# xiexh20/VisTracker

Measured on AMD Instinct MI355X. Metric: frames/sec joint SMPL+object fit, higher is better.
Workload: dtype f32 (decoder GEMMs: 22-bit split-f16 operands x3 MFMA, fp32 accumulate)

## Files before the change

include/vistracker.h:

```cpp
#ifndef VISTRACKER_H
#define VISTRACKER_H

#ifdef __cplusplus
extern "C" {
#endif

#define VT_OK 0
#define VT_ERR_ARG -1
#define VT_ERR_HIP -2
#define VT_ERR_BUSY -3

#define VT_SMPL_V 6890
#define VT_SMPL_J 52
#define VT_SMPL_NB 10
#define VT_SMPL_NP 459
#define VT_FEAT 611
#define VT_HID 128

const char *vt_last_error(void);
int vt_version(void);

typedef struct vt_smplh vt_smplh;

int vt_smplh_create(vt_smplh **out, const float *v_template, const float *shapedirs, const float *posedirs,
                    const float *J_regressor, const float *weights, const int *parents, void *stream);
void vt_smplh_destroy(vt_smplh *h);

long vt_smplh_workspace_floats(int B);

int vt_smplh_forward(const vt_smplh *h, const float *pose, const float *betas, const float *trans, int B,
                     float *verts, float *jtr, float *v_posed, float *ws, void *stream);

long vt_smplh_bwd_scratch_floats(int B);
int vt_smplh_backward(const vt_smplh *h, const float *pose, const float *betas, int B, const float *dverts,
                      const float *djtr, const float *v_posed, const float *ws, float *scratch,
                      float *dpose, float *dbetas, float *dtrans, void *stream);

int vt_rodrigues_forward(const float *aa, int n, float *R, void *stream);
int vt_rodrigues_backward(const float *aa, int n, const float *dR, float *daa, void *stream);

typedef struct vt_landmarks vt_landmarks;
int vt_landmarks_create(vt_landmarks **out, const int *indptr, const int *indices, const float *data, int K, int V,
                        void *stream);
void vt_landmarks_destroy(vt_landmarks *h);
int vt_landmarks_forward(const vt_landmarks *h, const float *verts, int B, float *out, void *stream);
int vt_landmarks_backward(const vt_landmarks *h, const float *dout, int B, float *dverts, int accumulate, void *stream);

int vt_mahalanobis(const float *x, int B, int stride, int off, int n, const float *mean, const float *prec,
                   float *value, float *dx, float gscale, void *stream);

int vt_fill_f64(double *p, long n, double value, void *stream);
int vt_sum_to_term(const float *value, int n, float scale, double *term, void *stream);

typedef struct vt_sifnet vt_sifnet;
int vt_sifnet_create(vt_sifnet **out, const float *const *w, const float *const *b, const float *cam, void *stream);
void vt_sifnet_destroy(vt_sifnet *h);

int vt_nchw_to_nhwc(const float *src, int B, int C, int H, int W, float *dst, void *stream);

typedef struct {
    const float *maps[8];
    int res[8];
    const float *proj;
    int proj_cols;
    int act_level;
    int proj_level;
    int force_fp32;
} vt_maps;

int vt_query_forward(const vt_sifnet *h, const vt_maps *maps, const float *pts, const float *crop_center,
                     const float *body_center, int B, int N,
                     float *df, float *pca, float *parts, float *centers, float *vis, void *stream);
int vt_query_backward(const vt_sifnet *h, const vt_maps *maps, const float *pts, const float *crop_center,
                      const float *body_center, int B, int N,
                      const float *d_df, const float *d_pca, const float *d_parts, const float *d_centers,
                      const float *d_vis, float *dpts, void *stream);

long vt_query_projection_floats(const vt_maps *maps, int B);
int vt_query_build_projection(const vt_sifnet *h, const vt_maps *maps, int B, float *proj, void *stream);

int vt_query_human_loss(const vt_sifnet *h, const vt_maps *maps, const float *pts, const float *crop_center,
                        const float *body_center, int B, int N, const int *labels, const int *order, float w_dfh, float w_part,
                        float *dpts, double *terms, void *stream);
int vt_query_object_loss(const vt_sifnet *h, const vt_maps *maps, const float *pts, const float *crop_center,
                         const float *body_center, int B, int N, const float *occ, float w_obj,
                         float *dpts, double *terms, void *stream);

typedef struct vt_conv3x3 vt_conv3x3;
int vt_conv3x3_create(vt_conv3x3 **out, const float *weight, int cout, int cin, void *stream);
void vt_conv3x3_destroy(vt_conv3x3 *h);
int vt_conv3x3_forward(const vt_conv3x3 *h, const float *in, int B, int H, int W, float *out, int out_cstride, int out_coff, void *stream);
int vt_conv3x3_forward_gn(const vt_conv3x3 *h, const float *in, int in_cstride, int in_coff, const float *gn_stats, const float *gamma,
                          const float *beta, int groups, int B, int H, int W, float *out, int out_cstride, int out_coff, void *stream);
int vt_conv3x3_forward_gn_stats(const vt_conv3x3 *h, const float *in, int in_cstride, int in_coff, const float *gn_stats, const float *gamma,
                                const float *beta, int groups, int B, int H, int W, float *out, int out_cstride, int out_coff, double *stats_ws,
                                int stats_groups, void *stream);
int vt_conv3x3_forward_block(const vt_conv3x3 *h, const float *in, int in_cstride, int in_coff, const float *gn_stats, const float *gamma,
                             const float *beta, int groups, int B, int H, int W, float *out, int out_cstride, int out_coff,
                             const float *res, int res_cstride, int res_coff, float *fin, int fin_cstride, int fin_coff,
                             double *stats_ws, int stats_groups, void *stream);
int vt_conv3x3_tiles(int H, int W);
typedef struct vt_stem7x7 vt_stem7x7;
int vt_stem7x7_create(vt_stem7x7 **out, const float *weight, const float *bias, int cout, int cin, void *stream);
void vt_stem7x7_destroy(vt_stem7x7 *h);
int vt_stem7x7_forward(const vt_stem7x7 *h, const float *in, int in_cstride, int in_coff, int B, int H, int W, float *out, int out_cstride, int out_coff, void *stream);
typedef struct vt_conv1x1 vt_conv1x1;
int vt_conv1x1_create(vt_conv1x1 **out, const float *weight, const float *bias, int cout, int cin, void *stream);
void vt_conv1x1_destroy(vt_conv1x1 *h);
int vt_conv1x1_forward(const vt_conv1x1 *h, const float *in, int in_cstride, int in_coff, const float *gn_stats, const float *gamma, const float *beta, int groups,
                       int B, int H, int W, float *out, int out_cstride, int out_coff, const float *res, int res_cstride, int res_coff,
                       double *stats_ws, int stats_groups, void *stream);
int vt_groupnorm_finalize(double *ws, int nblk, int B, int HW, int C, int groups, float eps, void *stream);
int vt_conv3x3_forward_block_stats(const vt_conv3x3 *h, const float *in, int in_cstride, int in_coff, const float *gn_stats, const float *gamma,
                                   const float *beta, int groups, int B, int H, int W, float *out, int out_cstride, int out_coff,
                                   const float *res, int res_cstride, int res_coff, float *fin, int fin_cstride, int fin_coff,
                                   double *stats_ws, int stats_groups, double *fin_stats_ws, int fin_stats_groups, void *stream);
int vt_avgpool2x2_stats(const float *x, int B, int H, int W, int C, float *out, double *stats_ws, int stats_groups, void *stream);
int vt_sweep_blocks(int HW);
int vt_groupnorm_stats(const float *x, int cstride, int coff, int B, int HW, int C, int groups, float eps, double *ws, void *stream);

#define VT_PRECISION_SPLIT_F16 0
#define VT_PRECISION_FP32 1
int vt_sifnet_set_precision(vt_sifnet *h, int mode);
int vt_sifnet_get_precision(const vt_sifnet *h);

int vt_query_set_human_kernel(int threads);

int vt_query_project_step(const vt_sifnet *h, const vt_maps *maps, const float *pts, const float *crop_center,
                          const float *body_center, int B, int N, int df_idx, float threshold, float *pts_out,
                          float *df_target, void *stream);

int vt_kpts_step(const vt_landmarks *h, const float *verts, const float *kpts, const float *crop_center, int B, int mode, const float *cam, float net_size,
                 float gscale, double *term, float *J, float *dverts, int accumulate, void *stream);
int vt_query_human_step(const vt_sifnet *h, const vt_maps *maps, const float *pts, const float *crop_center, const float *body_center,
                        int B, int N, const int *labels, const int *order, float w_dfh, float w_part, int accumulate, float w_accel,
                        double *term_accel, float *dpts, double *terms, void *stream);
int vt_objstep_head(const float *M0, const float *noise, const float *t, const float *s, int B, const float *X0_points, int N, float *X_points,
                    const float *X0_verts, int NV, float *X_verts, float *R, double *terms, int nzero, float *svd_ws, void *stream);
int vt_temporal_loss2(const float *v, int B, int D, float gscale_accel, double *term_accel, float gscale_velocity, double *term_velocity, float *dv,
                      int init_zero, void *stream);
int vt_objstep_tail(const float *X0_verts, int NV, const float *dX_verts, const float *X0_points, int N, const float *dX_points, const float *s, int B,
                    const float *M0, const float *noise, const float *t, const float *t_init, float w_trans, double *term_trans,
                    float *dR, float *dt, float *dM,
                    float *pR, float *mR, float *vR, float lrR, float *pT, float *mT, float *vT, float lrT, int adam_step, float beta1, float beta2, float eps,
                    double *terms, const float *w, int nterms, float tol, int armed, float *state, int *stop_flag, float *history, int slot, int *ticket, int nzero,
                    float *svd_ws, void *stream);
int vt_objstep_tail_temporal(const float *X_points, float gscale_accel, double *term_accel, float gscale_velocity, double *term_velocity, int init_zero,
                             const float *X0_verts, int NV, const float *dX_verts, const float *X0_points, int N, const float *dX_points, const float *s, int B,
                             const float *M0, const float *noise, const float *t, const float *t_init, float w_trans, double *term_trans,
                             float *dR, float *dt, float *dM,
                             float *pR, float *mR, float *vR, float lrR, float *pT, float *mT, float *vT, float lrT, int adam_step, float beta1, float beta2, float eps,
                             double *terms, const float *w, int nterms, float tol, int armed, float *state, int *stop_flag, float *history, int slot, int *ticket, int nzero,
                             float *svd_ws, void *stream);
int vt_smplstep_tail(float *pose, const float *pose_init, float *dpose, int B, const float *prior_mean, const float *prior_prec, float gscale_prior,
                     double *term_prior, float w_pinit, double *term_pinit,
                     float *p0, int ps0, const float *g0, int gs0, float *m0, float *v0, int n0, float lr0,
                     float *p1, int ps1, const float *g1, int gs1, float *m1, float *v1, int n1, float lr1,
                     float *p2, int ps2, const float *g2, int gs2, float *m2, float *v2, int n2, float lr2,
                     int adam_step, float beta1, float beta2, float eps,
                     double *terms, const float *w, int nterms, float tol, int armed, float *state, int *stop_flag, float *history, int slot, int *ticket, int nzero,
                     void *stream);

int vt_so3_project_forward(const float *M0, const float *noise, int B, float *R, void *stream);
int vt_so3_project_backward(const float *M0, const float *noise, int B, const float *dR, float *dM, void *stream);

int vt_rigid_forward(const float *X0, int shared_x0, const float *R, const float *t, const float *s, int B, int N,
                     float *X, void *stream);
int vt_rigid_backward(const float *X0, int shared_x0, const float *s, int B, int N, const float *dX,
                      float *dR, float *dt, int accumulate, void *stream);

int vt_accel_loss(const float *v, int B, int D, const float *elem_w, float gscale, double *term, float *dv, void *stream);
int vt_accel_loss_strided(const float *v, int B, int D, int stride, const float *elem_w, float gscale, double *term,
                          float *dv, void *stream);
int vt_velocity_loss(const float *v, int B, int D, float gscale, double *term, float *dv, void *stream);

int vt_kpts_loss(const float *J, const float *kpts, const float *crop_center, int B, int K, int mode,
                 const float *cam, float net_size, float gscale, double *term, float *dJ, void *stream);

int vt_sqdiff_loss(const float *a, int a_stride, const float *b, int b_stride, int rows, int cols, float denom,
                   float gscale, double *term, float *da, void *stream);

long vt_collision_workspace_bytes(int B, int n_smpl_faces);
int vt_collision_loss(const float *smpl_verts, int n_smpl_verts, const int *smpl_faces, int n_smpl_faces, const float *obj_verts, int n_obj_verts,
                      const int *obj_faces, int n_obj_faces, int B, float sigma, int max_collisions, float gscale, double *term,
                      float *d_obj_t, int *pairs_per_frame, void *workspace, void *stream);

int vt_chamfer_ragged(const float *x, const int *offx, const float *y, const int *offy, int P, float gscale,
                      double *term, float *dx, float *dy, void *stream);
long vt_chamfer_ws_bytes(long total_x, long total_y, int P);
int vt_chamfer_ragged_ws(const float *x, const int *offx, long total_x, const float *y, const int *offy, long total_y, int P, float gscale,
                         double *term, float *dx, float *dy, void *ws, void *stream);

int vt_chamfer_ragged_idx(const float *x, const int *offx, long total_x, const float *y_base, const int *idx_y, const int *offy, long total_y, int P,
                          float gscale, double *term, float *dy_base, void *ws, int run_plan, void *stream);

int vt_nn_distance(const float *query, int nq, const float *search, int ns, int P, float *dist, void *stream);

long vt_sil_workspace_floats(int B, int NV, int NF, int size);
int vt_sil_forward(const float *verts, int B, int NV, const int *faces, int NF, const float *K, int size,
                   float *image, int *face_index, float *ws, void *stream);
int vt_sil_backward(const float *verts, int B, int NV, const int *faces, int NF, const float *K, int size,
                    const int *face_index, const float *d_image, float eps, float *ws, float *dverts, void *stream);
int vt_sil_setup(const float *mask_h, const float *mask_o, int B, int H, int W, const float *crop_centers, double expansion, int out, double crop_size,
                 double net_size, const double *cam_norm, double image_width, float *image_ref, float *keep_mask, float *K, double *boxes_ws, void *stream);

int vt_sil_mask_loss(const float *image, const float *keep, const float *ref, const float *occ, int B, int size,
                     float gscale, double *term, float *per_frame, float *d_image, void *stream);

int vt_sil_step(const float *verts, int B, int NV, const int *faces, int NF, const float *K, int size, const float *keep, const float *ref,
                const float *occ, float gscale, float eps, double *term, int *face_index, float *d_image, float *ws, float *dverts, void *stream);

int vt_triplane_render(const float *verts, const float *center, int B, int NV, const int *faces, int NF, int size,
                       float *masks, int *face_index, float *ws, void *stream);

int vt_upsample2x_bicubic_add(const float *low, const float *skip, int B, int h, int w, int C, float *out, void *stream);
int vt_upsample2x_bicubic_add_stats(const float *low, const float *skip, int B, int h, int w, int C, float *out, double *stats_ws, int stats_groups,
                                    void *stream);

long vt_groupnorm_workspace_doubles(int B, int HW, int C, int groups);
int vt_groupnorm_nhwc(const float *x, const float *gamma, const float *beta, int B, int HW, int C, int groups, float eps,
                      int relu, double *ws, float *y, void *stream);

int vt_adam_step(float *p, const float *g, float *m, float *v, long n, int step, float lr, float beta1, float beta2,
                 float eps, const int *stop_flag, void *stream);

int vt_adam_step_2d(float *p, long p_stride, const float *g, long g_stride, float *m, float *v, int rows, int cols,
                    int step, float lr, float beta1, float beta2, float eps, const int *stop_flag, void *stream);

int vt_loss_reduce_and_stop(const double *terms, const float *w, int nterms, float tol, int armed, float *state,
                            int *stop_flag, float *history, int slot, void *stream);

int vt_fill(float *p, long n, float value, void *stream);

int vt_stream_set_skip_flag(void *stream, const int *flag);

int vt_gen_round_compact(const float *surface, const float *df_target, const float *pre, const unsigned char *active, int B, int S, float filter_val,
                         float zmin, const long long *fill, int cap, int write, float *buf_points, int *order, float *kept_pre, long long *cnt,
                         long long *fill_out, void *stream);
int vt_gen_scatter_heads(const float *pred, int B, int C, int kmax, const long long *fill_old, const long long *cnt, int cap, float *buf, void *stream);
int vt_gen_resample(const float *samples, const int *order, const long long *cnt, const float *init, int B, int S, int S0, const float *u,
                    const float *pert, int M, float near_scale, float *out, void *stream);

long vt_render_workspace_bytes(int B, int NF, int size, int anti_aliasing, long list_entries);
int vt_render_static_create(void **layer, const float *verts, int NV, const int *faces, int NS, const float *face_colors, const float *K, float orig_size,
                            const float *light, int size, int anti_aliasing, void *stream);
void vt_render_static_destroy(void *layer);
int vt_render_rgb(const float *verts, int B, int NV, const int *faces, int NF, const float *face_colors, const float *K, int k_per_view, float orig_size,
                  const float *light, const float *background, const void *static_layer, int size, int anti_aliasing, float *rgb, float *alpha, float *depth,
                  int *face_index, void *ws, long ws_bytes, long *list_entries, void *stream);
int vt_render_panel_u8(const float *rgb, int B, int size, int row0, int nrows, int col0, int ncols, unsigned char *out, const long long *view_off,
                       long long out_row_stride, void *stream);
int vt_render_rgb_pv(const float *verts, int B, int NV, const int *faces, int NF, const float *face_colors, int colors_per_view, const float *K, int k_per_view,
                     float orig_size, const float *light, const float *background, const void *static_layer, int size, int anti_aliasing, float *rgb,
                     float *alpha, float *depth, int *face_index, void *ws, long ws_bytes, long *list_entries, void *stream);

int vt_contact_regions(const float *smpl_verts, const int *labels, const float *obj_verts, int B, int NVs, int NVo, int P, float thres, int *nn_idx,
                       float *nn_dist, int *part, int *count, float *centre, void *stream);
int vt_contact_spheres(const float *centre, const int *count, int B, int P, const float *unit_verts, int NSV, float radius, float *out, void *stream);
int vt_contact_face_colors(const int *part, int B, int NVo, const int *obj_faces, int NFo, int face_off, const float *base_colors, int NF, const float *palette,
                           int P, float *out, void *stream);

long vt_jpeg_workspace_bytes(int n, int H, int W, int subsampling, long long *max_out_bytes);
int vt_jpeg_encode(const unsigned char *rgb, int n, int H, int W, long long frame_stride, long long row_stride, int quality, int subsampling, void *ws,
                   long ws_bytes, unsigned char *out, long long out_cap, long long *offsets, void *stream);

int vt_query_set_clock_probe(unsigned long long *counters);
long vt_calibrate_workspace_bytes(void);
int vt_calibrate(void *work, double *out, void *stream);

#ifdef __cplusplus
}
#endif
#endif
```

vistracker_amd/_lib.py:

```python
from __future__ import annotations

import ctypes as C
import os

_HERE = os.path.dirname(os.path.abspath(__file__))
LIB_PATH = os.environ.get("VT_LIB_PATH", os.path.join(_HERE, "libvistracker_hip.so"))

vp = C.c_void_p
fp = C.c_void_p
ci = C.c_int
cl = C.c_long
cf = C.c_float
cd = C.c_double


class VtMaps(C.Structure):
    _fields_ = [("maps", C.c_void_p * 8), ("res", C.c_int * 8), ("proj", C.c_void_p), ("proj_cols", C.c_int),
                ("act_level", C.c_int), ("proj_level", C.c_int), ("force_fp32", C.c_int)]


SIGNATURES = {
    "vt_last_error": (C.c_char_p, []),
    "vt_version": (ci, []),
    "vt_smplh_create": (ci, [C.POINTER(vp), vp, vp, vp, vp, vp, vp, vp]),
    "vt_smplh_destroy": (None, [vp]),
    "vt_smplh_workspace_floats": (cl, [ci]),
    "vt_smplh_bwd_scratch_floats": (cl, [ci]),
    "vt_smplh_forward": (ci, [vp, fp, fp, fp, ci, fp, fp, fp, fp, vp]),
    "vt_smplh_backward": (ci, [vp, fp, fp, ci, fp, fp, fp, fp, fp, fp, fp, fp, vp]),
    "vt_rodrigues_forward": (ci, [fp, ci, fp, vp]),
    "vt_rodrigues_backward": (ci, [fp, ci, fp, fp, vp]),
    "vt_landmarks_create": (ci, [C.POINTER(vp), vp, vp, vp, ci, ci, vp]),
    "vt_landmarks_destroy": (None, [vp]),
    "vt_landmarks_forward": (ci, [vp, fp, ci, fp, vp]),
    "vt_landmarks_backward": (ci, [vp, fp, ci, fp, ci, vp]),
    "vt_mahalanobis": (ci, [fp, ci, ci, ci, ci, fp, fp, fp, fp, cf, vp]),
    "vt_fill_f64": (ci, [fp, cl, cd, vp]),
    "vt_sum_to_term": (ci, [fp, ci, cf, fp, vp]),
    "vt_sifnet_create": (ci, [C.POINTER(vp), C.POINTER(vp), C.POINTER(vp), vp, vp]),
    "vt_sifnet_destroy": (None, [vp]),
    "vt_nchw_to_nhwc": (ci, [fp, ci, ci, ci, ci, fp, vp]),
    "vt_query_forward": (ci, [vp, C.POINTER(VtMaps), fp, fp, fp, ci, ci, fp, fp, fp, fp, fp, vp]),
    "vt_query_backward": (ci, [vp, C.POINTER(VtMaps), fp, fp, fp, ci, ci, fp, fp, fp, fp, fp, fp, vp]),
    "vt_query_human_loss": (ci, [vp, C.POINTER(VtMaps), fp, fp, fp, ci, ci, fp, fp, cf, cf, fp, fp, vp]),
    "vt_query_object_loss": (ci, [vp, C.POINTER(VtMaps), fp, fp, fp, ci, ci, fp, cf, fp, fp, vp]),
    "vt_query_set_human_kernel": (ci, [ci]),
    "vt_sifnet_set_precision": (ci, [vp, ci]),
    "vt_sifnet_get_precision": (ci, [vp]),
    "vt_groupnorm_nhwc": (ci, [fp, fp, fp, ci, ci, ci, ci, cf, ci, fp, fp, vp]),
    "vt_upsample2x_bicubic_add": (ci, [fp, fp, ci, ci, ci, ci, fp, vp]),
    "vt_conv3x3_create": (ci, [C.POINTER(vp), vp, ci, ci, vp]),
    "vt_conv3x3_destroy": (None, [vp]),
    "vt_conv3x3_forward": (ci, [vp, fp, ci, ci, ci, fp, ci, ci, vp]),
    "vt_conv3x3_forward_gn": (ci, [vp, fp, ci, ci, fp, fp, fp, ci, ci, ci, ci, fp, ci, ci, vp]),
    "vt_groupnorm_stats": (ci, [fp, ci, ci, ci, ci, ci, ci, cf, fp, vp]),
    "vt_groupnorm_workspace_doubles": (C.c_long, [ci, ci, ci, ci]),
    "vt_groupnorm_finalize": (ci, [fp, ci, ci, ci, ci, ci, cf, vp]),
    "vt_conv3x3_tiles": (ci, [ci, ci]),
    "vt_kpts_step": (ci, [vp, fp, fp, fp, ci, ci, vp, cf, cf, fp, fp, fp, ci, vp]),
    "vt_query_human_step": (ci, [vp, C.POINTER(VtMaps), fp, fp, fp, ci, ci, fp, fp, cf, cf, ci, cf, fp, fp, fp, vp]),
    "vt_objstep_head": (ci, [fp, fp, fp, fp, ci, fp, ci, fp, fp, ci, fp, fp, fp, ci, fp, vp]),
    "vt_temporal_loss2": (ci, [fp, ci, ci, cf, fp, cf, fp, fp, ci, vp]),
    "vt_objstep_tail": (ci, [fp, ci, fp, fp, ci, fp, fp, ci, fp, fp, fp, fp, cf, fp, fp, fp, fp,
                             fp, fp, fp, cf, fp, fp, fp, cf, ci, cf, cf, cf,
                             fp, vp, ci, cf, ci, fp, fp, fp, ci, fp, ci, fp, vp]),
    "vt_objstep_tail_temporal": (ci, [fp, cf, fp, cf, fp, ci,
                                      fp, ci, fp, fp, ci, fp, fp, ci, fp, fp, fp, fp, cf, fp, fp, fp, fp,
                                      fp, fp, fp, cf, fp, fp, fp, cf, ci, cf, cf, cf,
                                      fp, vp, ci, cf, ci, fp, fp, fp, ci, fp, ci, fp, vp]),
    "vt_smplstep_tail": (ci, [fp, fp, fp, ci, fp, fp, cf, fp, cf, fp,
                              fp, ci, fp, ci, fp, fp, ci, cf, fp, ci, fp, ci, fp, fp, ci, cf, fp, ci, fp, ci, fp, fp, ci, cf, ci, cf, cf, cf,
                              fp, vp, ci, cf, ci, fp, fp, fp, ci, fp, ci, vp]),
    "vt_stream_set_skip_flag": (ci, [vp, vp]),
    "vt_conv1x1_create": (ci, [C.POINTER(vp), vp, vp, ci, ci, vp]),
    "vt_stem7x7_create": (ci, [C.POINTER(vp), vp, vp, ci, ci, vp]),
    "vt_stem7x7_destroy": (None, [vp]),
    "vt_stem7x7_forward": (ci, [vp, fp, ci, ci, ci, ci, ci, fp, ci, ci, vp]),
    "vt_conv1x1_destroy": (None, [vp]),
    "vt_conv1x1_forward": (ci, [vp, fp, ci, ci, fp, fp, fp, ci, ci, ci, ci, fp, ci, ci, fp, ci, ci, fp, ci, vp]),
    "vt_conv3x3_forward_block": (ci, [vp, fp, ci, ci, fp, fp, fp, ci, ci, ci, ci, fp, ci, ci, fp, ci, ci, fp, ci, ci, fp, ci, vp]),
    "vt_conv3x3_forward_block_stats": (ci, [vp, fp, ci, ci, fp, fp, fp, ci, ci, ci, ci, fp, ci, ci, fp, ci, ci, fp, ci, ci, fp, ci, fp, ci, vp]),
    "vt_avgpool2x2_stats": (ci, [fp, ci, ci, ci, ci, fp, fp, ci, vp]),
    "vt_sweep_blocks": (ci, [ci]),
    "vt_upsample2x_bicubic_add_stats": (ci, [fp, fp, ci, ci, ci, ci, fp, fp, ci, vp]),
    "vt_conv3x3_forward_gn_stats": (ci, [vp, fp, ci, ci, fp, fp, fp, ci, ci, ci, ci, fp, ci, ci, fp, ci, vp]),
    "vt_triplane_render": (ci, [fp, fp, ci, ci, fp, ci, ci, fp, fp, fp, vp]),
    "vt_query_project_step": (ci, [vp, C.POINTER(VtMaps), fp, fp, fp, ci, ci, ci, cf, fp, fp, vp]),
    "vt_query_projection_floats": (C.c_long, [C.POINTER(VtMaps), ci]),
    "vt_query_build_projection": (ci, [vp, C.POINTER(VtMaps), ci, fp, vp]),
    "vt_so3_project_forward": (ci, [fp, fp, ci, fp, vp]),
    "vt_so3_project_backward": (ci, [fp, fp, ci, fp, fp, vp]),
    "vt_rigid_forward": (ci, [fp, ci, fp, fp, fp, ci, ci, fp, vp]),
    "vt_rigid_backward": (ci, [fp, ci, fp, ci, ci, fp, fp, fp, ci, vp]),
    "vt_accel_loss": (ci, [fp, ci, ci, fp, cf, fp, fp, vp]),
    "vt_accel_loss_strided": (ci, [fp, ci, ci, ci, fp, cf, fp, fp, vp]),
    "vt_velocity_loss": (ci, [fp, ci, ci, cf, fp, fp, vp]),
    "vt_kpts_loss": (ci, [fp, fp, fp, ci, ci, ci, vp, cf, cf, fp, fp, vp]),
    "vt_sqdiff_loss": (ci, [fp, ci, fp, ci, ci, ci, cf, cf, fp, fp, vp]),
    "vt_chamfer_ragged": (ci, [fp, fp, fp, fp, ci, cf, fp, fp, fp, vp]),
    "vt_chamfer_ws_bytes": (C.c_long, [C.c_long, C.c_long, ci]),
    "vt_chamfer_ragged_ws": (ci, [fp, fp, C.c_long, fp, fp, C.c_long, ci, cf, fp, fp, fp, fp, vp]),
    "vt_chamfer_ragged_idx": (ci, [fp, fp, C.c_long, fp, fp, fp, C.c_long, ci, cf, fp, fp, fp, ci, vp]),
    "vt_collision_workspace_bytes": (cl, [ci, ci]),
    "vt_collision_loss": (ci, [fp, ci, fp, ci, fp, ci, fp, ci, ci, cf, ci, cf, fp, fp, fp, fp, vp]),
    "vt_nn_distance": (ci, [fp, ci, fp, ci, ci, fp, vp]),
    "vt_sil_workspace_floats": (cl, [ci, ci, ci, ci]),
    "vt_sil_forward": (ci, [fp, ci, ci, fp, ci, fp, ci, fp, fp, fp, vp]),
    "vt_sil_backward": (ci, [fp, ci, ci, fp, ci, fp, ci, fp, fp, cf, fp, fp, vp]),
    "vt_sil_mask_loss": (ci, [fp, fp, fp, fp, ci, ci, cf, fp, fp, fp, vp]),
    "vt_sil_step": (ci, [fp, ci, ci, fp, ci, fp, ci, fp, fp, fp, cf, cf, fp, fp, fp, fp, fp, vp]),
    "vt_gen_round_compact": (ci, [fp, fp, fp, vp, ci, ci, cf, cf, vp, ci, ci, fp, vp, fp, vp, vp, vp]),
    "vt_gen_scatter_heads": (ci, [fp, ci, ci, ci, vp, vp, ci, fp, vp]),
    "vt_gen_resample": (ci, [fp, vp, vp, fp, ci, ci, ci, fp, fp, ci, cf, fp, vp]),
    "vt_sil_setup": (ci, [fp, fp, ci, ci, ci, fp, C.c_double, ci, C.c_double, C.c_double, C.POINTER(C.c_double), C.c_double, fp, fp, fp, fp, vp]),
    "vt_adam_step": (ci, [fp, fp, fp, fp, cl, ci, cf, cf, cf, cf, fp, vp]),
    "vt_adam_step_2d": (ci, [fp, cl, fp, cl, fp, fp, ci, ci, ci, cf, cf, cf, cf, fp, vp]),
    "vt_loss_reduce_and_stop": (ci, [fp, vp, ci, cf, ci, fp, fp, fp, ci, vp]),
    "vt_fill": (ci, [fp, cl, cf, vp]),
    "vt_selftest_mfma": (ci, [fp, fp, fp, vp]),
    "vt_query_set_clock_probe": (ci, [vp]),
    "vt_render_workspace_bytes": (cl, [ci, ci, ci, ci, cl]),
    "vt_render_static_create": (ci, [C.POINTER(vp), fp, ci, fp, ci, fp, fp, cf, C.POINTER(cf), ci, ci, vp]),
    "vt_render_static_destroy": (None, [vp]),
    "vt_render_rgb": (ci, [fp, ci, ci, fp, ci, fp, fp, ci, cf, C.POINTER(cf), C.POINTER(cf), vp, ci, ci, fp, fp, fp, fp, fp, cl,
                           C.POINTER(cl), vp]),
    "vt_render_panel_u8": (ci, [fp, ci, ci, ci, ci, ci, ci, fp, fp, C.c_longlong, vp]),
    "vt_render_rgb_pv": (ci, [fp, ci, ci, fp, ci, fp, ci, fp, ci, cf, C.POINTER(cf), C.POINTER(cf), vp, ci, ci, fp, fp, fp, fp, fp, cl,
                              C.POINTER(cl), vp]),
    "vt_contact_regions": (ci, [fp, fp, fp, ci, ci, ci, ci, cf, fp, fp, fp, fp, fp, vp]),
    "vt_contact_spheres": (ci, [fp, fp, ci, ci, fp, ci, cf, fp, vp]),
    "vt_contact_face_colors": (ci, [fp, ci, ci, fp, ci, ci, fp, ci, fp, ci, fp, vp]),
    "vt_jpeg_workspace_bytes": (cl, [ci, ci, ci, ci, C.POINTER(C.c_longlong)]),
    "vt_jpeg_encode": (ci, [fp, ci, ci, ci, C.c_longlong, C.c_longlong, ci, ci, vp, cl, vp, C.c_longlong,
                            C.POINTER(C.c_longlong), vp]),
    "vt_calibrate_workspace_bytes": (cl, []),
    "vt_calibrate": (ci, [vp, C.POINTER(C.c_double), vp]),
}

_lib = None


class VtError(RuntimeError):
    pass


def lib():
    global _lib
    if _lib is None:
        if not os.path.exists(LIB_PATH):
            raise VtError(f"{LIB_PATH} is missing: build it with `make -C vistracker_amd/csrc` "
                          f"(or `python -c 'import __graft_entry__ as g; g.build()'`); there is no CPU fallback")
        import torch
        l = C.CDLL(LIB_PATH)
        for name, (res, args) in SIGNATURES.items():
            fn = getattr(l, name)
            fn.restype = res
            fn.argtypes = args
        _lib = l
        _host_tuning()
    return _lib


def _host_tuning():
    if os.environ.get("VT_HOST_THP", "keep") != "off":
        return
    try:
        C.CDLL(None, use_errno=True).prctl(41, 1, 0, 0, 0)
    except Exception:
        pass


VT_OK, VT_ERR_ARG, VT_ERR_HIP, VT_ERR_BUSY = 0, -1, -2, -3


def check(rc: int):
    if rc != 0:
        raise VtError(f"libvistracker_hip error {rc}: {lib().vt_last_error().decode()}")


def stream_ptr():
    import torch
    return torch.cuda.current_stream().cuda_stream


def dptr(t):
    if t is None:
        return None
    if not t.is_cuda:
        raise VtError("libvistracker_hip ops need CUDA (HIP) tensors; there is no CPU fallback in the product path")
    if not t.is_contiguous():
        raise VtError("libvistracker_hip ops need contiguous tensors")
    import torch
    if t.device.index != torch.cuda.current_device():
        raise VtError(f"tensor on cuda:{t.device.index} but the current device is cuda:{torch.cuda.current_device()}: "
                      "wrap the call in `with torch.cuda.device(tensor.device):`")
    return t.data_ptr()
```

vistracker_amd/csrc/smplh.hip:

```cpp
#include "common.h"
#include <cstring>

#define V_ VT_SMPL_V
#define J_ VT_SMPL_J
#define NB_ VT_SMPL_NB
#define NP_ VT_SMPL_NP
#define VP_ 6912
#define NVT_ 27
#define KQ_ 472
#define NQ_ 480
typedef float f32x4 __attribute__((ext_vector_type(4)));
#define MFMA16(a, b, c) __builtin_amdgcn_mfma_f32_16x16x4f32((a), (b), (c), 0, 0, 0)

#define WS_R 0
#define WS_J (52 * 9)
#define WS_G (WS_J + 52 * 3)
#define WS_A (WS_G + 52 * 12)
#define WS_FRAME (WS_A + 52 * 12)
#define PT_DA 0
#define PT_DTR 624
#define PT_N 627
#define KTOT_ (VP_ * 3)
#define KG_SLAB 24
#define NKS_ (KTOT_ / 16 / KG_SLAB)

#define SCHED_STEPS 32
#define SCHED_WIDTH 10
struct SmplParents { int p[J_]; int nsteps; short sched[SCHED_STEPS][SCHED_WIDTH]; };

#define SP_K 8
struct vt_smplh {
    float *Q_kcv, *Q_t, *W_jv, *W_v64, *J_t, *J_s;
    float *W_sp;
    int nnz;
    SmplParents par;
};

struct RodCtx { float n, ax, ay, az, c, s, qn, w, x, y, z; };

__device__ __forceinline__ void rodrigues_fwd(const float *t, float *R, RodCtx *k)
{
    const float xe = t[0] + 1e-8f, ye = t[1] + 1e-8f, ze = t[2] + 1e-8f;
    const float n = sqrtf(xe * xe + ye * ye + ze * ze);
    const float ax = t[0] / n, ay = t[1] / n, az = t[2] / n;
    const float h = n * 0.5f;
    const float c = cosf(h), s = sinf(h);
    const float q0 = c, q1 = s * ax, q2 = s * ay, q3 = s * az;
    const float qn = sqrtf(q0 * q0 + q1 * q1 + q2 * q2 + q3 * q3);
    const float w = q0 / qn, x = q1 / qn, y = q2 / qn, z = q3 / qn;
    const float w2 = w * w, x2 = x * x, y2 = y * y, z2 = z * z;
    const float wx = w * x, wy = w * y, wz = w * z, xy = x * y, xz = x * z, yz = y * z;
    R[0] = w2 + x2 - y2 - z2; R[1] = 2 * xy - 2 * wz;   R[2] = 2 * wy + 2 * xz;
    R[3] = 2 * wz + 2 * xy;   R[4] = w2 - x2 + y2 - z2; R[5] = 2 * yz - 2 * wx;
    R[6] = 2 * xz - 2 * wy;   R[7] = 2 * wx + 2 * yz;   R[8] = w2 - x2 - y2 + z2;
    if (k) { k->n = n; k->ax = ax; k->ay = ay; k->az = az; k->c = c; k->s = s; k->qn = qn; k->w = w; k->x = x; k->y = y; k->z = z; }
}

__device__ __forceinline__ void rodrigues_bwd(const float *t, const float *dR, float *dt)
{
    float R[9]; RodCtx k; rodrigues_fwd(t, R, &k);
    const float w = k.w, x = k.x, y = k.y, z = k.z;
    const float dw = 2 * w * (dR[0] + dR[4] + dR[8]) + 2 * (-z * dR[1] + y * dR[2] + z * dR[3] - x * dR[5] - y * dR[6] + x * dR[7]);
    const float dx = 2 * x * (dR[0] - dR[4] - dR[8]) + 2 * (y * dR[1] + z * dR[2] + y * dR[3] - w * dR[5] + z * dR[6] + w * dR[7]);
    const float dy = 2 * y * (-dR[0] + dR[4] - dR[8]) + 2 * (x * dR[1] + w * dR[2] + x * dR[3] + z * dR[5] - w * dR[6] + z * dR[7]);
    const float dz = 2 * z * (-dR[0] - dR[4] + dR[8]) + 2 * (-w * dR[1] + x * dR[2] + w * dR[3] + y * dR[5] + x * dR[6] + y * dR[7]);
    const float dot = w * dw + x * dx + y * dy + z * dz;
    const float dq0 = (dw - w * dot) / k.qn, dq1 = (dx - x * dot) / k.qn, dq2 = (dy - y * dot) / k.qn, dq3 = (dz - z * dot) / k.qn;
    const float dh = -k.s * dq0 + k.c * (k.ax * dq1 + k.ay * dq2 + k.az * dq3);
    const float dax = k.s * dq1, day = k.s * dq2, daz = k.s * dq3;
    const float dn = 0.5f * dh - (t[0] * dax + t[1] * day + t[2] * daz) / (k.n * k.n);
    dt[0] = dax / k.n + dn * (t[0] + 1e-8f) / k.n;
    dt[1] = day / k.n + dn * (t[1] + 1e-8f) / k.n;
    dt[2] = daz / k.n + dn * (t[2] + 1e-8f) / k.n;
}

__global__ void rodrigues_fwd_kernel(const float *aa, int n, float *R)
{
    const int i = blockIdx.x * blockDim.x + threadIdx.x;
    if (i >= n) return;
    float t[3] = {aa[3 * i], aa[3 * i + 1], aa[3 * i + 2]}, r[9];
    rodrigues_fwd(t, r, nullptr);
#pragma unroll
    for (int e = 0; e < 9; e++) R[9 * i + e] = r[e];
}

__global__ void rodrigues_bwd_kernel(const float *aa, int n, const float *dR, float *daa)
{
    const int i = blockIdx.x * blockDim.x + threadIdx.x;
    if (i >= n) return;
    float t[3] = {aa[3 * i], aa[3 * i + 1], aa[3 * i + 2]}, g[9], d[3];
#pragma unroll
    for (int e = 0; e < 9; e++) g[e] = dR[9 * i + e];
    rodrigues_bwd(t, g, d);
    daa[3 * i] = d[0]; daa[3 * i + 1] = d[1]; daa[3 * i + 2] = d[2];
}

__global__ __launch_bounds__(64) void smplh_pose_kernel(const float *__restrict__ pose, const float *__restrict__ betas,
                                                        const float *__restrict__ trans, const float *__restrict__ J_t,
                                                        const float *__restrict__ J_s, SmplParents par,
                                                        float *__restrict__ ws, float *__restrict__ jtr, const int *skip)
{
    VT_SKIP_RETURN(skip);
    __shared__ float sR[J_ * 9], sJ[J_ * 3], sG[J_ * 12];
    const int b = blockIdx.x, j = threadIdx.x;
    float *w = ws + (size_t)b * WS_FRAME;
    if (j < J_) {
        float t[3] = {pose[(b * J_ + j) * 3], pose[(b * J_ + j) * 3 + 1], pose[(b * J_ + j) * 3 + 2]}, R[9];
        rodrigues_fwd(t, R, nullptr);
#pragma unroll
        for (int e = 0; e < 9; e++) { sR[j * 9 + e] = R[e]; w[WS_R + j * 9 + e] = R[e]; }
#pragma unroll
        for (int c = 0; c < 3; c++) {
            float a = J_t[j * 3 + c];
#pragma unroll
            for (int l = 0; l < NB_; l++) a += J_s[(j * 3 + c) * NB_ + l] * betas[b * NB_ + l];
            sJ[j * 3 + c] = a; w[WS_J + j * 3 + c] = a;
        }
    }
    __shared__ int sPar[J_];
    if (j < J_) sPar[j] = par.p[j];
    __syncthreads();
    int lvl = 0, maxl = 0;
    if (j < J_) { for (int q = j; q != 0; q = sPar[q]) lvl++; }
    maxl = lvl;
    for (int o = 32; o > 0; o >>= 1) maxl = max(maxl, __shfl_xor(maxl, o, 64));
    maxl = __builtin_amdgcn_readfirstlane(maxl);
    if (j == 0) { for (int r = 0; r < 3; r++) { for (int c = 0; c < 3; c++) sG[r * 4 + c] = sR[r * 3 + c]; sG[r * 4 + 3] = sJ[r]; } }
    __syncthreads();
    for (int l = 1; l <= maxl; l++) {
        if (j < J_ && lvl == l) {
            const int i = j, p = sPar[i];
            const float *Gp = sG + 12 * p, *Ri = sR + 9 * i;
            const float d0 = sJ[3 * i] - sJ[3 * p], d1 = sJ[3 * i + 1] - sJ[3 * p + 1], d2 = sJ[3 * i + 2] - sJ[3 * p + 2];
            float *Gi = sG + 12 * i;
            for (int r = 0; r < 3; r++) {
                const float g0 = Gp[r * 4], g1 = Gp[r * 4 + 1], g2 = Gp[r * 4 + 2];
                Gi[r * 4 + 0] = g0 * Ri[0] + g1 * Ri[3] + g2 * Ri[6];
                Gi[r * 4 + 1] = g0 * Ri[1] + g1 * Ri[4] + g2 * Ri[7];
                Gi[r * 4 + 2] = g0 * Ri[2] + g1 * Ri[5] + g2 * Ri[8];
                Gi[r * 4 + 3] = g0 * d0 + g1 * d1 + g2 * d2 + Gp[r * 4 + 3];
            }
        }
        __syncthreads();
    }
    if (j < J_) {
        const float *G = sG + 12 * j;
#pragma unroll
        for (int r = 0; r < 3; r++) {
            const float gt = G[r * 4 + 3];
            w[WS_G + j * 12 + r * 4 + 0] = G[r * 4]; w[WS_G + j * 12 + r * 4 + 1] = G[r * 4 + 1];
            w[WS_G + j * 12 + r * 4 + 2] = G[r * 4 + 2]; w[WS_G + j * 12 + r * 4 + 3] = gt;
            w[WS_A + j * 12 + r * 4 + 0] = G[r * 4]; w[WS_A + j * 12 + r * 4 + 1] = G[r * 4 + 1]; w[WS_A + j * 12 + r * 4 + 2] = G[r * 4 + 2];
            w[WS_A + j * 12 + r * 4 + 3] = gt - (G[r * 4] * sJ[3 * j] + G[r * 4 + 1] * sJ[3 * j + 1] + G[r * 4 + 2] * sJ[3 * j + 2]);
            if (jtr) jtr[(b * J_ + j) * 3 + r] = gt + trans[3 * b + r];
        }
    }
}

#define FWD_FB 16
#ifndef FWD_PF
#define FWD_PF 6
#endif
#define AXS 516
#define SAS 628
#define FWD_R0 (FWD_FB * AXS > 8 * SAS ? FWD_FB * AXS : 8 * SAS)
__global__ __launch_bounds__(256) void smplh_verts_kernel(const float *__restrict__ Q_kcv, const float *__restrict__ W_jv,
                                                          const float *__restrict__ betas, const float *__restrict__ trans,
                                                          const float *__restrict__ ws, int B,
                                                          float *__restrict__ verts, float *__restrict__ v_posed, const float *__restrict__ W_sp, int nnz, const int *skip)
{
    VT_SKIP_RETURN(skip);
    extern __shared__ __attribute__((aligned(16))) float lds[];
    float *sAx = lds;
    float *sA = lds;
    float *sVp = lds + FWD_R0;
    float *sW = sVp + FWD_FB * 64 * 3;
    float *sTr = sW + (nnz > 0 ? 2 * SP_K * 64 : J_ * 64);
    const int tid = threadIdx.x, wave = tid >> 6, lane = tid & 63, q = lane >> 4, j = lane & 15;
    const int b0 = blockIdx.y * FWD_FB, v = blockIdx.x * 64 + wave * 16 + j;
    for (int k = tid; k < KQ_; k += 256) {
        const int e9 = k % 9;
        const float sub = (k < NP_ && (e9 == 0 || e9 == 4 || e9 == 8)) ? 1.f : 0.f;
        float val[FWD_FB];
#pragma unroll
        for (int f = 0; f < FWD_FB; f++) {
            const int b = min(b0 + f, B - 1);
            if (k < NP_) val[f] = ws[(size_t)b * WS_FRAME + WS_R + 9 + k];
            else if (k < NP_ + NB_) val[f] = betas[b * NB_ + (k - NP_)];
            else val[f] = (k == NP_ + NB_) ? 1.f : 0.f;
        }
#pragma unroll
        for (int f = 0; f < FWD_FB; f++) sAx[f * AXS + k] = val[f] - sub;
    }
    if (nnz > 0) {
        for (int i = tid; i < nnz * 64; i += 256) {
            sW[i] = W_sp[(size_t)(i >> 6) * VP_ + blockIdx.x * 64 + (i & 63)];
            sW[SP_K * 64 + i] = W_sp[(size_t)(SP_K + (i >> 6)) * VP_ + blockIdx.x * 64 + (i & 63)];
        }
    } else
        for (int i = tid; i < J_ * 64; i += 256) sW[i] = W_jv[(i >> 6) * VP_ + blockIdx.x * 64 + (i & 63)];
    if (tid < FWD_FB * 3) { const int f = tid / 3, b = min(b0 + f, B - 1); sTr[tid] = trans[b * 3 + tid % 3]; }
    __syncthreads();

    f32x4 acc[3];
#pragma unroll
    for (int c = 0; c < 3; c++) acc[c] = (f32x4){0.f, 0.f, 0.f, 0.f};
    constexpr int NS = KQ_ / 8;
    float bq[FWD_PF][2][3];
#define FWD_LOADQ(slot_, s_)                                                                     \
    {                                                                                            \
        const float *qk = Q_kcv + (size_t)(8 * (s_) + 2 * q) * 3 * VP_ + v;                      \
        _Pragma("unroll") for (int e = 0; e < 2; e++)                                            \
            _Pragma("unroll") for (int c = 0; c < 3; c++) bq[slot_][e][c] = qk[(size_t)(e * 3 + c) * VP_]; \
    }
#pragma unroll
    for (int s = 0; s < FWD_PF; s++) FWD_LOADQ(s, s)
#pragma unroll
    for (int s = 0; s < NS; s++) {
        const float2 av = *reinterpret_cast<const float2 *>(sAx + j * AXS + 8 * s + 2 * q);
#pragma unroll
        for (int c = 0; c < 3; c++) acc[c] = MFMA16(av.x, bq[s % FWD_PF][0][c], acc[c]);
#pragma unroll
        for (int c = 0; c < 3; c++) acc[c] = MFMA16(av.y, bq[s % FWD_PF][1][c], acc[c]);
        if (s + FWD_PF < NS) FWD_LOADQ(s % FWD_PF, s + FWD_PF)
        __builtin_amdgcn_sched_barrier(0);
    }
#undef FWD_LOADQ
    __syncthreads();
#pragma unroll
    for (int r = 0; r < 4; r++)
#pragma unroll
        for (int c = 0; c < 3; c++) sVp[((4 * q + r) * 64 + wave * 16 + j) * 3 + c] = acc[c][r];
    const int vv = tid & 63, vg = blockIdx.x * 64 + vv;
#pragma unroll 1
    for (int r = 0; r < 4; r++) {
        if ((r & 1) == 0) {
            if (r) __syncthreads();
            for (int i = tid; i < 8 * 624; i += 256) {
                const int sl = i / 624, f = 4 * (sl >> 1) + r + (sl & 1), b = min(b0 + f, B - 1);
                sA[sl * SAS + (i % 624)] = ws[(size_t)b * WS_FRAME + WS_A + (i % 624)];
            }
            __syncthreads();
        }
        const int f = 4 * wave + r, b = b0 + f;
        float T[12];
#pragma unroll
        for (int e = 0; e < 12; e++) T[e] = 0.f;
        const float4 *Af = reinterpret_cast<const float4 *>(sA + (2 * wave + (r & 1)) * SAS);
        if (nnz > 0) {
            for (int k = 0; k < nnz; k++) {
                const int jj = __float_as_int(sW[k * 64 + vv]);
                const float wj = sW[(SP_K + k) * 64 + vv];
                const float4 a0 = Af[jj * 3], a1 = Af[jj * 3 + 1], a2 = Af[jj * 3 + 2];
                T[0] += wj * a0.x; T[1] += wj * a0.y; T[2] += wj * a0.z; T[3] += wj * a0.w;
                T[4] += wj * a1.x; T[5] += wj * a1.y; T[6] += wj * a1.z; T[7] += wj * a1.w;
                T[8] += wj * a2.x; T[9] += wj * a2.y; T[10] += wj * a2.z; T[11] += wj * a2.w;
            }
        } else {
#pragma unroll 4
            for (int jj = 0; jj < J_; jj++) {
                const float wj = sW[jj * 64 + vv];
                const float4 a0 = Af[jj * 3], a1 = Af[jj * 3 + 1], a2 = Af[jj * 3 + 2];
                T[0] += wj * a0.x; T[1] += wj * a0.y; T[2] += wj * a0.z; T[3] += wj * a0.w;
                T[4] += wj * a1.x; T[5] += wj * a1.y; T[6] += wj * a1.z; T[7] += wj * a1.w;
                T[8] += wj * a2.x; T[9] += wj * a2.y; T[10] += wj * a2.z; T[11] += wj * a2.w;
            }
        }
        if (b < B && vg < V_) {
            const float p0 = sVp[(f * 64 + vv) * 3], p1 = sVp[(f * 64 + vv) * 3 + 1], p2 = sVp[(f * 64 + vv) * 3 + 2];
            const size_t o = ((size_t)b * V_ + vg) * 3;
#pragma unroll
            for (int rr = 0; rr < 3; rr++) verts[o + rr] = T[rr * 4] * p0 + T[rr * 4 + 1] * p1 + T[rr * 4 + 2] * p2 + T[rr * 4 + 3] + sTr[f * 3 + rr];
            v_posed[o] = p0; v_posed[o + 1] = p1; v_posed[o + 2] = p2;
        }
    }
}

template <int FB>
__global__ __launch_bounds__(256) void smplh_bwd_tile_kernel(const float *__restrict__ W_v64, const float *__restrict__ ws,
                                                             const float *__restrict__ v_posed, const float *__restrict__ dverts,
                                                             int B, float *__restrict__ part, float *__restrict__ dvp_g, const int *skip)
{
    VT_SKIP_RETURN(skip);
    extern __shared__ __attribute__((aligned(16))) float lds[];
    float *sdT = lds;
    float *sA = sdT + 256 * 13;
    const int tid = threadIdx.x, tile = blockIdx.x, b0 = blockIdx.y * FB, v0 = tile * 256, v = v0 + tid;
    const int wave = tid >> 6, lane = tid & 63, q = lane >> 4, j = lane & 15;
    for (int i = tid; i < FB * 624; i += 256) { const int f = i / 624, b = min(b0 + f, B - 1); sA[i] = ws[(size_t)b * WS_FRAME + WS_A + (i % 624)]; }
    float w1[4][13], w2[64];
#pragma unroll
    for (int mt = 0; mt < 4; mt++)
#pragma unroll
        for (int ks = 0; ks < 13; ks++) w1[mt][ks] = W_v64[(size_t)(v0 + 64 * wave + 16 * mt + j) * 64 + 4 * ks + q];
#pragma unroll
    for (int ks = 0; ks < 64; ks++) w2[ks] = W_v64[(size_t)(v0 + 4 * ks + q) * 64 + wave * 16 + j];
    __syncthreads();
    float dvn[3] = {0.f, 0.f, 0.f}, vpn[3] = {0.f, 0.f, 0.f};
    auto fetch = [&](int b) {
#pragma unroll
        for (int r = 0; r < 3; r++) { dvn[r] = 0.f; vpn[r] = 0.f; }
        if (b < B && v < V_) {
            const size_t o = ((size_t)b * V_ + v) * 3;
            dvn[0] = dverts[o]; dvn[1] = dverts[o + 1]; dvn[2] = dverts[o + 2];
            vpn[0] = v_posed[o]; vpn[1] = v_posed[o + 1]; vpn[2] = v_posed[o + 2];
        }
    };
    fetch(b0);
#pragma unroll 1
    for (int f = 0; f < FB; f++) {
        const int b = b0 + f;
        const float dv[3] = {dvn[0], dvn[1], dvn[2]}, vp[3] = {vpn[0], vpn[1], vpn[2]};
        if (f + 1 < FB) fetch(b + 1);
#pragma unroll
        for (int r = 0; r < 3; r++) {
            sdT[tid * 13 + r * 4 + 0] = dv[r] * vp[0]; sdT[tid * 13 + r * 4 + 1] = dv[r] * vp[1];
            sdT[tid * 13 + r * 4 + 2] = dv[r] * vp[2]; sdT[tid * 13 + r * 4 + 3] = dv[r];
        }
        __syncthreads();
        {
            f32x4 t[4];
#pragma unroll
            for (int mt = 0; mt < 4; mt++) t[mt] = (f32x4){0.f, 0.f, 0.f, 0.f};
#pragma unroll
            for (int ks = 0; ks < 13; ks++) {
                const float bv = j < 12 ? sA[f * 624 + (4 * ks + q) * 12 + j] : 0.f;
#pragma unroll
                for (int mt = 0; mt < 4; mt++) t[mt] = MFMA16(w1[mt][ks], bv, t[mt]);
            }
            const int r4 = (j < 12 ? (j >> 2) : 0) * 4 + 3;
#pragma unroll
            for (int mt = 0; mt < 4; mt++) {
#pragma unroll
                for (int r = 0; r < 4; r++) {
                    const int vl = 64 * wave + 16 * mt + 4 * q + r;
                    float x = t[mt][r] * sdT[vl * 13 + r4];
                    x += __shfl_down(x, 4, 16) + __shfl_down(x, 8, 16);
                    if (j < 3 && b < B) dvp_g[(size_t)b * KTOT_ + (size_t)(v0 + vl) * 3 + j] = x;
                }
            }
        }
        {
            f32x4 acc = (f32x4){0.f, 0.f, 0.f, 0.f}, acc2 = (f32x4){0.f, 0.f, 0.f, 0.f};
#pragma unroll
            for (int ks = 0; ks < 64; ks += 2) {
                const int va = 4 * ks + q, vb = va + 4;
                const float a0 = j < 12 ? sdT[va * 13 + j] : 0.f, a1 = j < 12 ? sdT[vb * 13 + j] : 0.f;
                acc = MFMA16(a0, w2[ks], acc);
                acc2 = MFMA16(a1, w2[ks + 1], acc2);
            }
            acc += acc2;
            if (b < B) {
                float *dst = part + ((size_t)tile * B + b) * PT_N;
                const int jn = wave * 16 + j;
#pragma unroll
                for (int r = 0; r < 4; r++) {
                    const int e = 4 * q + r;
                    if (e < 12) {
                        if (jn < J_) dst[PT_DA + jn * 12 + e] = acc[r];
                        else if (jn == J_ && (e & 3) == 3) dst[PT_DTR + (e >> 2)] = acc[r];
                    }
                }
            }
        }
        __syncthreads();
    }
}

#define BL_M 96
#ifndef BL_NW
#define BL_NW 1
#endif
#define BL_AS 132
__global__ __launch_bounds__(256) void smplh_bwd_blend_kernel(const float *__restrict__ Q_p, const float *__restrict__ dvp_g, int B,
                                                              float *__restrict__ part3, const int *skip)
{
    VT_SKIP_RETURN(skip);
    __shared__ __attribute__((aligned(16))) float sA[BL_M * BL_AS];
    const int tid = threadIdx.x, wave = tid >> 6, lane = tid & 63, q = lane >> 4, j = lane & 15;
    const int ks = blockIdx.x, m0 = blockIdx.z * BL_M, nt0 = blockIdx.y * (4 * BL_NW) + wave * BL_NW;
    f32x4 acc[6][BL_NW];
#pragma unroll
    for (int mt = 0; mt < 6; mt++)
#pragma unroll
        for (int n = 0; n < BL_NW; n++) acc[mt][n] = (f32x4){0.f, 0.f, 0.f, 0.f};
    const float4 *Q4 = reinterpret_cast<const float4 *>(Q_p);
#pragma unroll 1
    for (int c = 0; c < KG_SLAB / 8; c++) {
        __syncthreads();
        for (int i = tid; i < BL_M * 32; i += 256) {
            const int row = i >> 5, c4 = i & 31, b = m0 + row;
            float4 v = make_float4(0.f, 0.f, 0.f, 0.f);
            if (b < B) v = *reinterpret_cast<const float4 *>(dvp_g + (size_t)b * KTOT_ + (size_t)(ks * KG_SLAB + c * 8) * 16 + c4 * 4);
            *reinterpret_cast<float4 *>(sA + row * BL_AS + c4 * 4) = v;
        }
        __syncthreads();
#pragma unroll
        for (int g = 0; g < 8; g++) {
            const size_t kg = (size_t)ks * KG_SLAB + c * 8 + g;
            float bq[BL_NW][4];
#pragma unroll
            for (int n = 0; n < BL_NW; n++) {
                const float4 fq = Q4[(kg * (NQ_ / 16) + min(nt0 + n, NQ_ / 16 - 1)) * 64 + lane];
                bq[n][0] = fq.x; bq[n][1] = fq.y; bq[n][2] = fq.z; bq[n][3] = fq.w;
            }
#pragma unroll
            for (int mt = 0; mt < 6; mt++) {
                const float4 a4 = *reinterpret_cast<const float4 *>(sA + (mt * 16 + j) * BL_AS + g * 16 + q * 4);
                const float av[4] = {a4.x, a4.y, a4.z, a4.w};
#pragma unroll
                for (int s = 0; s < 4; s++)
#pragma unroll
                    for (int n = 0; n < BL_NW; n++) acc[mt][n] = MFMA16(av[s], bq[n][s], acc[mt][n]);
            }
        }
    }
#pragma unroll
    for (int mt = 0; mt < 6; mt++) {
#pragma unroll
        for (int r = 0; r < 4; r++) {
            const int b = m0 + mt * 16 + 4 * q + r;
            if (b < B) {
                float *dst = part3 + ((size_t)ks * B + b) * NQ_;
#pragma unroll
                for (int n = 0; n < BL_NW; n++)
                    if (nt0 + n < NQ_ / 16) dst[(nt0 + n) * 16 + j] = acc[mt][n][r];
            }
        }
    }
}

__global__ __launch_bounds__(256) void smplh_bwd_frame_kernel(const float *__restrict__ pose, const float *__restrict__ J_s,
                                                              SmplParents par, const float *__restrict__ ws,
                                                              const float *__restrict__ part, const float *__restrict__ part3,
                                                              const float *__restrict__ djtr, int B, float *__restrict__ dpose, float *__restrict__ dbetas,
                                                              float *__restrict__ dtrans, const int *skip)
{
    VT_SKIP_RETURN(skip);
    __shared__ float red[PT_N], red3[NQ_];
    __shared__ float sdG[J_ * 12], sdJ[J_ * 3], sdR[J_ * 9];
    __shared__ float sG[J_ * 12], sRm[J_ * 9], sJr[J_ * 3];
    const int b = blockIdx.x, tid = threadIdx.x;
    const float *w = ws + (size_t)b * WS_FRAME;
    for (int i = tid; i < J_ * 12; i += 256) sG[i] = w[WS_G + i];
    for (int i = tid; i < J_ * 9; i += 256) sRm[i] = w[WS_R + i];
    for (int i = tid; i < J_ * 3; i += 256) sJr[i] = w[WS_J + i];
    for (int i = tid; i < PT_N; i += 256) {
        float s = 0.f;
#pragma unroll 9
        for (int t = 0; t < NVT_; t++) s += part[((size_t)t * B + b) * PT_N + i];
        red[i] = s;
    }
    for (int i = tid; i < NQ_; i += 256) {
        float s = 0.f;
#pragma unroll 9
        for (int t = 0; t < NKS_; t++) s += part3[((size_t)t * B + b) * NQ_ + i];
        red3[i] = s;
    }
    __syncthreads();
    if (tid < J_) {
        const int j = tid;
        const float *G = sG + 12 * j; const float *Jr = sJr;
        float dj[3] = {0.f, 0.f, 0.f};
#pragma unroll
        for (int r = 0; r < 3; r++) {
            const float dat = red[PT_DA + 12 * j + r * 4 + 3];
#pragma unroll
            for (int c = 0; c < 3; c++) { sdG[12 * j + r * 4 + c] = red[PT_DA + 12 * j + r * 4 + c] - dat * Jr[3 * j + c]; dj[c] -= G[r * 4 + c] * dat; }
            sdG[12 * j + r * 4 + 3] = dat + (djtr ? djtr[(b * J_ + j) * 3 + r] : 0.f);
        }
        sdJ[3 * j] = dj[0]; sdJ[3 * j + 1] = dj[1]; sdJ[3 * j + 2] = dj[2];
#pragma unroll
        for (int e = 0; e < 9; e++) sdR[9 * j + e] = 0.f;
    }
    __syncthreads();
    const int jloc = tid / 24, el = tid - 24 * jloc;
    const int nsteps = par.nsteps > 0 ? par.nsteps : J_ - 1;
    for (int step = 0; step < nsteps; step++) {
        const int j = par.nsteps > 0 ? (jloc < SCHED_WIDTH ? (int)par.sched[step][jloc < SCHED_WIDTH ? jloc : 0] : -1) : (jloc == 0 ? J_ - 1 - step : -1);
        if (j >= 1) {
            const int p = par.p[j];
            const float *Gp = sG + 12 * p, *Rj = sRm + 9 * j, *dGj = sdG + 12 * j;
            float upd = 0.f; float *dst = nullptr; float upd2 = 0.f; float *dst2 = nullptr;
            if (el < 12) {
                const int r = el >> 2, c = el & 3;
                dst = sdG + 12 * p + el;
                if (c < 3) upd = dGj[r * 4] * Rj[3 * c] + dGj[r * 4 + 1] * Rj[3 * c + 1] + dGj[r * 4 + 2] * Rj[3 * c + 2] + dGj[r * 4 + 3] * (sJr[3 * j + c] - sJr[3 * p + c]);
                else upd = dGj[r * 4 + 3];
            } else if (el < 21) {
                const int e = el - 12, r = e / 3, c = e - 3 * r;
                dst = sdR + 9 * j + e;
                upd = Gp[r] * dGj[c] + Gp[4 + r] * dGj[4 + c] + Gp[8 + r] * dGj[8 + c];
            } else {
                const int c = el - 21;
                upd = Gp[c] * dGj[3] + Gp[4 + c] * dGj[7] + Gp[8 + c] * dGj[11];
                dst = sdJ + 3 * j + c; dst2 = sdJ + 3 * p + c; upd2 = -upd;
            }
            if (dst) *dst += upd;
            if (dst2) *dst2 += upd2;
        }
        __syncthreads();
    }
    if (tid < 3) { for (int c = 0; c < 3; c++) sdR[3 * tid + c] += sdG[tid * 4 + c]; sdJ[tid] += sdG[tid * 4 + 3]; }
    __syncthreads();
    if (tid < J_) {
        const int j = tid;
        float g[9], t[3] = {pose[(b * J_ + j) * 3], pose[(b * J_ + j) * 3 + 1], pose[(b * J_ + j) * 3 + 2]}, d[3];
#pragma unroll
        for (int e = 0; e < 9; e++) g[e] = sdR[9 * j + e] + (j >= 1 ? red3[(j - 1) * 9 + e] : 0.f);
        rodrigues_bwd(t, g, d);
        dpose[(b * J_ + j) * 3] = d[0]; dpose[(b * J_ + j) * 3 + 1] = d[1]; dpose[(b * J_ + j) * 3 + 2] = d[2];
    } else if (tid >= 64 && tid < 64 + NB_) {
        const int l = tid - 64;
        float s = red3[NP_ + l];
        for (int i = 0; i < J_ * 3; i++) s += J_s[i * NB_ + l] * sdJ[i];
        dbetas[b * NB_ + l] = s;
    } else if (tid >= 128 && tid < 131) {
        const int c = tid - 128;
        float s = red[PT_DTR + c];
        if (djtr) for (int j = 0; j < J_; j++) s += djtr[(b * J_ + j) * 3 + c];
        dtrans[b * 3 + c] = s;
    }
}

extern "C" int vt_smplh_create(vt_smplh **out, const float *v_template, const float *shapedirs, const float *posedirs,
                               const float *J_regressor, const float *weights, const int *parents, void *stream)
{
    VT_REQUIRE(out && v_template && shapedirs && posedirs && J_regressor && weights && parents, "vt_smplh_create: null argument");
    hipStream_t st = vt_stream(stream);
    vt_smplh *h = new vt_smplh();
    for (int j = 0; j < J_; j++) h->par.p[j] = (j == 0) ? 0 : parents[j];
    for (int j = 1; j < J_; j++) VT_REQUIRE(h->par.p[j] >= 0 && h->par.p[j] < j, "vt_smplh_create: parents[%d]=%d must be in [0,%d)", j, parents[j], j);
    {
        int lvl[J_], rank[J_], maxl = 0;
        lvl[0] = 0; rank[0] = 0;
        for (int j = 1; j < J_; j++) { lvl[j] = lvl[h->par.p[j]] + 1; maxl = std::max(maxl, lvl[j]); rank[j] = 0; for (int k = j + 1; k < J_; k++) rank[j] += (h->par.p[k] == h->par.p[j]); }
        int n = 0; bool ok = true;
        for (int t = 0; t < SCHED_STEPS; t++) for (int i = 0; i < SCHED_WIDTH; i++) h->par.sched[t][i] = -1;
        for (int l = maxl; l >= 1 && ok; l--)
            for (int r = 0; r < J_ && ok; r++) {
                int cnt = 0;
                for (int j = J_ - 1; j >= 1; j--) if (lvl[j] == l && rank[j] == r) { if (n >= SCHED_STEPS || cnt >= SCHED_WIDTH) { ok = false; break; } h->par.sched[n][cnt++] = (short)j; }
                if (cnt) n++;
            }
        h->par.nsteps = ok ? n : 0;
    }
    float *Q_kcv = new float[(size_t)KQ_ * 3 * VP_](), *Q_t = new float[(size_t)VP_ * 3 * NQ_](), *W_jv = new float[(size_t)J_ * VP_](),
          *J_t = new float[J_ * 3], *J_s = new float[J_ * 3 * NB_];
    for (int v = 0; v < V_; v++) for (int c = 0; c < 3; c++) {
        for (int k = 0; k < NP_ + NB_ + 1; k++) {
            const float val = k < NP_ ? posedirs[((size_t)v * 3 + c) * NP_ + k]
                            : (k < NP_ + NB_ ? shapedirs[((size_t)v * 3 + c) * NB_ + (k - NP_)] : v_template[v * 3 + c]);
            Q_kcv[(size_t)(k * 3 + c) * VP_ + v] = val;
            {
                const size_t kr = (size_t)v * 3 + c, g = kr >> 4, qq = (kr & 15) >> 2, ss = kr & 3;
                Q_t[((g * (NQ_ / 16) + (k >> 4)) * 64 + qq * 16 + (k & 15)) * 4 + ss] = val;
            }
        }
    }
    float *W_v64 = new float[(size_t)VP_ * 64]();
    for (int v = 0; v < V_; v++) { for (int j = 0; j < J_; j++) { W_jv[(size_t)j * VP_ + v] = weights[(size_t)v * J_ + j]; W_v64[(size_t)v * 64 + j] = weights[(size_t)v * J_ + j]; } W_v64[(size_t)v * 64 + J_] = 1.0f; }
    float *W_sp = new float[(size_t)2 * SP_K * VP_]();
    int nnz = 0;
    for (int v = 0; v < V_; v++) {
        int k = 0;
        for (int j = 0; j < J_; j++) {
            const float w = weights[(size_t)v * J_ + j];
            if (w == 0.0f) continue;
            if (k < SP_K) { const int jj = j; memcpy(&W_sp[(size_t)k * VP_ + v], &jj, 4); W_sp[(size_t)(SP_K + k) * VP_ + v] = w; }
            k++;
        }
        nnz = k > nnz ? k : nnz;
    }
    h->nnz = nnz <= SP_K ? (nnz > 0 ? nnz : 1) : 0;
    for (int j = 0; j < J_; j++) for (int c = 0; c < 3; c++) {
        double a = 0; double sb[NB_] = {0};
        for (int v = 0; v < V_; v++) {
            const double r = J_regressor[(size_t)j * V_ + v];
            if (r == 0.0) continue;
            a += r * v_template[v * 3 + c];
            for (int l = 0; l < NB_; l++) sb[l] += r * shapedirs[((size_t)v * 3 + c) * NB_ + l];
        }
        J_t[j * 3 + c] = (float)a;
        for (int l = 0; l < NB_; l++) J_s[(j * 3 + c) * NB_ + l] = (float)sb[l];
    }
    int rc = VT_OK;
    if ((rc = vt_upload(&h->Q_kcv, Q_kcv, (size_t)KQ_ * 3 * VP_, st)) || (rc = vt_upload(&h->Q_t, Q_t, (size_t)VP_ * 3 * NQ_, st)) ||
        (rc = vt_upload(&h->W_jv, W_jv, (size_t)J_ * VP_, st)) || (rc = vt_upload(&h->W_v64, W_v64, (size_t)VP_ * 64, st)) ||
        (rc = vt_upload(&h->J_t, J_t, (size_t)J_ * 3, st)) || (rc = vt_upload(&h->J_s, J_s, (size_t)J_ * 3 * NB_, st)) ||
        (rc = vt_upload(&h->W_sp, W_sp, (size_t)2 * SP_K * VP_, st))) {
        return rc;
    }
    VT_HIP(hipStreamSynchronize(st));
    delete[] Q_kcv; delete[] Q_t; delete[] W_jv; delete[] W_v64; delete[] J_t; delete[] J_s; delete[] W_sp;
    *out = h;
    return VT_OK;
}

extern "C" void vt_smplh_destroy(vt_smplh *h)
{
    if (!h) return;
    hipFree(h->Q_kcv); hipFree(h->Q_t); hipFree(h->W_jv); hipFree(h->W_v64); hipFree(h->J_t); hipFree(h->J_s); hipFree(h->W_sp);
    delete h;
}

extern "C" long vt_smplh_workspace_floats(int B) { return (long)B * WS_FRAME; }
extern "C" long vt_smplh_bwd_scratch_floats(int B) { return (long)NVT_ * B * PT_N + (long)B * KTOT_ + (long)NKS_ * B * NQ_; }

#define BWD_FB 6

extern "C" int vt_smplh_forward(const vt_smplh *h, const float *pose, const float *betas, const float *trans, int B,
                                float *verts, float *jtr, float *v_posed, float *ws, void *stream)
{
    VT_REQUIRE(h && pose && betas && trans && verts && v_posed && ws && B > 0, "vt_smplh_forward: null argument or B <= 0");
    hipStream_t st = vt_stream(stream); const int *skip = vt_skip_flag_of(st);
    hipLaunchKernelGGL(smplh_pose_kernel, dim3(B), dim3(64), 0, st, pose, betas, trans, h->J_t, h->J_s, h->par, ws, jtr, skip);
    VT_LAUNCH_CHECK();
    const size_t lds_f = sizeof(float) * (FWD_R0 + FWD_FB * 64 * 3 + (h->nnz > 0 ? 2 * SP_K * 64 : J_ * 64) + FWD_FB * 3);
    VT_LDS_LIMIT(smplh_verts_kernel, sizeof(float) * (FWD_R0 + FWD_FB * 64 * 3 + J_ * 64 + FWD_FB * 3));
    hipLaunchKernelGGL(smplh_verts_kernel, dim3(VP_ / 64, (B + FWD_FB - 1) / FWD_FB), dim3(256), lds_f, st, h->Q_kcv, h->W_jv, betas, trans, ws, B,
                       verts, v_posed, h->W_sp, h->nnz, skip);
    VT_LAUNCH_CHECK();
    return VT_OK;
}

extern "C" int vt_smplh_backward(const vt_smplh *h, const float *pose, const float *betas, int B, const float *dverts,
                                 const float *djtr, const float *v_posed, const float *ws, float *scratch,
                                 float *dpose, float *dbetas, float *dtrans, void *stream)
{
    (void)betas;
    VT_REQUIRE(h && pose && dverts && v_posed && ws && scratch && dpose && dbetas && dtrans && B > 0, "vt_smplh_backward: null argument or B <= 0");
    hipStream_t st = vt_stream(stream); const int *skip = vt_skip_flag_of(st);
    const size_t lds = sizeof(float) * (256 * 13 + BWD_FB * 624);
    float *dvp_g = scratch + (size_t)NVT_ * B * PT_N, *part3 = dvp_g + (size_t)B * KTOT_;
    VT_LDS_LIMIT(smplh_bwd_tile_kernel<BWD_FB>, lds);
    hipLaunchKernelGGL(smplh_bwd_tile_kernel<BWD_FB>, dim3(NVT_, (B + BWD_FB - 1) / BWD_FB), dim3(256), lds, st, h->W_v64, ws, v_posed, dverts, B, scratch, dvp_g, skip);
    VT_LAUNCH_CHECK();
    hipLaunchKernelGGL(smplh_bwd_blend_kernel, dim3(NKS_, (NQ_ / 16 + 4 * BL_NW - 1) / (4 * BL_NW), (B + BL_M - 1) / BL_M), dim3(256), 0, st, h->Q_t, dvp_g, B, part3, skip);
    VT_LAUNCH_CHECK();
    hipLaunchKernelGGL(smplh_bwd_frame_kernel, dim3(B), dim3(256), 0, st, pose, h->J_s, h->par, ws, scratch, part3, djtr, B, dpose, dbetas, dtrans, skip);
    VT_LAUNCH_CHECK();
    return VT_OK;
}

extern "C" int vt_rodrigues_forward(const float *aa, int n, float *R, void *stream)
{
    VT_REQUIRE(aa && R && n > 0, "vt_rodrigues_forward: bad argument");
    hipLaunchKernelGGL(rodrigues_fwd_kernel, dim3((n + 255) / 256), dim3(256), 0, vt_stream(stream), aa, n, R);
    VT_LAUNCH_CHECK();
    return VT_OK;
}

extern "C" int vt_rodrigues_backward(const float *aa, int n, const float *dR, float *daa, void *stream)
{
    VT_REQUIRE(aa && dR && daa && n > 0, "vt_rodrigues_backward: bad argument");
    hipLaunchKernelGGL(rodrigues_bwd_kernel, dim3((n + 255) / 256), dim3(256), 0, vt_stream(stream), aa, n, dR, daa);
    VT_LAUNCH_CHECK();
    return VT_OK;
}
```

vistracker_amd/fitting.py:

```python
from __future__ import annotations

import contextlib
import ctypes as C
import functools
import os
import threading
import time
from dataclasses import dataclass, field

import numpy as np
import torch

from . import _lib as L
from . import ops

FIT_WEIGHTS = {"pose": 1e-5, "hand": 1e-5, "j2d": 0.09, "object": 900.0, "part": 0.0025, "contact": 900.0, "scale": 100.0,
               "df_h": 100.0, "mask": 0.0009, "ocent": 0.0, "pinit": 25.0, "rot": 100.0, "trans": 100.0,
               "stemp": 10000.0, "otemp": 225.0, "ovtemp": 2500.0, "collide": 9.0}
SMPLT_WEIGHTS = {"pose": 1e-5, "hand": 1e-5, "kpts": 0.09, "temp": 900.0, "ptemp": 25.0, "pinit": 900.0}
JOINT_WEIGHTS_66 = np.repeat(np.array([1, 10, 10, 10, 5, 5, 10, 1, 1, 10, 1, 1, 5, 5, 5, 5, 5, 5, 1, 1, 1, 1], np.float32), 3)
JOINT_WEIGHTS_66[37:39] = 10.0


def _lib():
    return L.lib()


def _chk(rc):
    L.check(rc)


def _ev_begin(prof):
    if prof is None:
        return None
    e = torch.cuda.Event(enable_timing=True); e.record()
    return e


def _flush_events(prof, local, executed):
    if prof is None:
        return
    for k, v in local.items():
        prof[k].extend((a, b, n) for a, b, n, step in v if executed is None or step < executed)


def _ev_end(prof, key, e0, frames, step):
    if prof is None:
        return
    e1 = torch.cuda.Event(enable_timing=True); e1.record()
    prof[key].append((e0, e1, frames, step))


class Terms:

    def __init__(self, names, device):
        self.names = list(names)
        self.buf = torch.zeros(len(self.names), dtype=torch.float64, device=device)
        self.idx = {n: i for i, n in enumerate(self.names)}

    def ptr(self, name):
        return self.buf.data_ptr() + 8 * self.idx[name]

    def zero(self, first=0, count=None):
        count = len(self.names) - first if count is None else count
        _chk(_lib().vt_fill_f64(self.buf.data_ptr() + 8 * first, count, 0.0, L.stream_ptr()))

    def weights(self, table, decay, extra=None):
        w = np.zeros(16, np.float32)
        for n, i in self.idx.items():
            w[i] = table[n] / (1.0 + decay) * (1.0 if extra is None else extra.get(n, 1.0))
        return w


class AdamState:

    def __init__(self, slices, stop_flag):
        self.slices = slices
        self.m = [torch.zeros(p.shape[0], n, device=p.device) for p, n, g, lr in slices]
        self.v = [torch.zeros(p.shape[0], n, device=p.device) for p, n, g, lr in slices]
        self.t = 0
        self.stop_flag = stop_flag

    def tick(self):
        self.t += 1
        return self.t

    def step(self):
        t = self.tick()
        for (p, n, g, lr), m, v in zip(self.slices, self.m, self.v):
            _chk(_lib().vt_adam_step_2d(p.data_ptr(), p.shape[1], g.data_ptr(), g.shape[1], m.data_ptr(), v.data_ptr(), p.shape[0], n,
                                        t, lr, 0.9, 0.999, 1e-8, self.stop_flag.data_ptr(), L.stream_ptr()))

    @functools.cached_property
    def smpl_tail_groups(self):
        out = ()
        for (p, n, g, lr), m, v in zip(self.slices, self.m, self.v):
            out += (p.data_ptr(), p.shape[1], g.data_ptr(), g.shape[1], m.data_ptr(), v.data_ptr(), n, lr)
        return out + (None, 0, None, 0, None, None, 0, 0.0) * (3 - len(self.slices))

    @functools.cached_property
    def object_tail_groups(self):
        rot = trans = (None, None, None, 0.0)
        for (p, n, g, lr), m, v in zip(self.slices, self.m, self.v):
            if n == 9:
                rot = (p.data_ptr(), m.data_ptr(), v.data_ptr(), lr)
            else:
                trans = (p.data_ptr(), m.data_ptr(), v.data_ptr(), lr)
        return rot + trans


def _check_finite(res, what):
    executed = res.losses[:res.steps]
    if executed.size and not np.isfinite(executed).all():
        bad = int(np.flatnonzero(~np.isfinite(executed))[0])
        raise FloatingPointError(f"{what}: non-finite loss at Adam step {bad} (non-finite input or decoder activation out of range)")


def _as_input(t, dev):
    if t is None:
        return None
    return torch.as_tensor(t).to(device=dev, dtype=torch.float32).contiguous()


def _require_params(*ts):
    for t in ts:
        if not (torch.is_tensor(t) and t.is_cuda and t.dtype == torch.float32 and t.is_contiguous()):
            raise L.VtError("fit loops update their parameters in place: pass contiguous float32 CUDA tensors "
                            f"(got {type(t).__name__} {getattr(t, 'dtype', None)} on {getattr(t, 'device', None)})")
        if t.device != ts[0].device:
            raise L.VtError("fit loops: all parameters must live on the same device")


@dataclass
class FitResult:
    steps: int = 0
    outer_iters: int = 0
    stopped_early: bool = False
    losses: np.ndarray = field(default_factory=lambda: np.zeros(0, np.float32))


def morton_order(points) -> np.ndarray:
    p = np.asarray(points, np.float64)
    q = ((p - p.min(0)) / (p.max(0) - p.min(0) + 1e-12) * 1023).astype(np.int64)

    def part(x):
        x = (x | (x << 16)) & 0x030000FF; x = (x | (x << 8)) & 0x0300F00F; x = (x | (x << 4)) & 0x030C30C3
        return (x | (x << 2)) & 0x09249249
    return np.argsort(part(q[:, 0]) | (part(q[:, 1]) << 1) | (part(q[:, 2]) << 2), kind="stable")


def morton_order_device(p: torch.Tensor) -> torch.Tensor:
    p = p.double()
    lo = p.min(0).values; hi = p.max(0).values
    q = ((p - lo) / (hi - lo + 1e-12) * 1023).long()

    def part(x):
        x = (x | (x << 16)) & 0x030000FF; x = (x | (x << 8)) & 0x0300F00F; x = (x | (x << 4)) & 0x030C30C3
        return (x | (x << 2)) & 0x09249249
    key = part(q[:, 0]) | (part(q[:, 1]) << 1)
    if p.shape[1] > 2:
        key = key | (part(q[:, 2]) << 2)
    return torch.argsort(key, stable=True).to(torch.int32)


class _StopWatch:
    _tls = threading.local()

    def __init__(self, ctx, stop, lookahead):
        self.ctx, self.stop, self.look = ctx, stop, lookahead
        self.pending = None; self.n = 0
        if lookahead:
            pool = getattr(self._tls, "pool", None)
            if pool is None or pool[0] != stop.device:
                pool = (stop.device, torch.zeros(2, dtype=torch.int32).pin_memory(), [torch.cuda.Event(), torch.cuda.Event()])
                self._tls.pool = pool
            _, self.host, self.ev = pool

    def _wait(self, k):
        t0 = time.perf_counter()
        self.ev[k].synchronize()
        with self.ctx._counter_lock:
            self.ctx.host_wait_s += time.perf_counter() - t0
        return bool(int(self.host[k]))

    def check(self):
        if not self.look:
            return bool(self.ctx._read_stop(self.stop))
        k = self.n & 1; self.n += 1
        self.host[k:k + 1].copy_(self.stop, non_blocking=True); self.ev[k].record()
        prev, self.pending = self.pending, k
        return prev is not None and self._wait(prev)

    def final(self):
        if not self.look or self.pending is None:
            return False
        k, self.pending = self.pending, None
        return self._wait(k)


class _Fit:

    def __init__(self, dev, names, nsteps, prev_loss, prof):
        self.terms = Terms(names, dev)
        self.stop = torch.zeros(1, dtype=torch.int32, device=dev)
        self.loss_state = torch.full((2,), prev_loss, device=dev)
        self.ticket = torch.zeros(1, dtype=torch.int32, device=dev)
        self.hist = torch.full((nsteps,), float("nan"), device=dev)
        self.lp = {"human": [], "object": []} if prof is not None else None
        self.adam = None


class _SmplFit(_Fit):

    def __init__(self, pose, betas, trans, names, nsteps, prev_loss, prof=None):
        dev = pose.device; B = self.B = pose.shape[0]
        super().__init__(dev, names, nsteps, prev_loss, prof)
        self.pose, self.betas, self.trans = pose, betas, trans
        self.verts = torch.empty(B, 6890, 3, device=dev); self.jtr = torch.empty(B, 52, 3, device=dev); self.vposed = torch.empty_like(self.verts)
        self.ws = torch.empty(_lib().vt_smplh_workspace_floats(B), device=dev); self.scratch = torch.empty(_lib().vt_smplh_bwd_scratch_floats(B), device=dev)
        self.dverts = torch.empty_like(self.verts); self.J = torch.empty(B, 25, 3, device=dev); self.dJ = torch.empty_like(self.J)
        self.dpose = torch.empty(B, 156, device=dev); self.dbetas = torch.empty(B, 10, device=dev); self.dtrans = torch.empty(B, 3, device=dev)
        self.vb = torch.empty(B, device=dev)
        self.pose_init = pose.clone()

    @property
    def vert_order_ptr(self):
        return self.vert_order.data_ptr() if self.vert_order is not None else None


class _ObjectFit(_Fit):

    def __init__(self, ctx, obj_R, obj_t, sil, nsteps, prof):
        dev = obj_R.device; B = self.B = obj_R.shape[0]; N = self.N = ctx.obj_points.shape[0]; NV = self.NV = ctx.obj_verts.shape[0]
        super().__init__(dev, ["object", "otemp", "ovtemp", "mask", "trans", "contact", "collide", "scale"], nsteps, 300.0, prof)
        self.obj_R, self.obj_t, self.sil = obj_R, obj_t, sil
        self.R = torch.empty(B, 3, 3, device=dev); self.X = torch.empty(B, N, 3, device=dev); self.dX = torch.empty_like(self.X)
        self.svd_ws = torch.empty(B, 22, device=dev)
        self.dR = torch.empty(B, 3, 3, device=dev); self.dM = torch.empty(B, 3, 3, device=dev); self.dt = torch.empty(B, 3, device=dev)
        if sil is not None:
            self.Vt = torch.empty(B, NV, 3, device=dev); self.dVt = torch.empty_like(self.Vt)
            self.fidx = torch.empty(B, sil.size, sil.size, dtype=torch.int32, device=dev); self.dimg = torch.empty(B, sil.size, sil.size, device=dev)
            self.sws = torch.empty(_lib().vt_sil_workspace_floats(B, NV, ctx.obj_faces.shape[0], sil.size), device=dev)
            if not ctx.fused_steps:
                self.img = torch.empty_like(self.dimg); self.per = torch.empty(B, device=dev)
        self.trans_init = None
        self.Vc = self.cws = None
        self.contact = None


class FitContext:
    use_projection = True
    sort_object_points = True
    sort_query_points = True
    collision_loss = False
    fused_steps = os.environ.get("VT_FUSED_STEPS", "1") != "0"
    fused_smpl_query = os.environ.get("VT_FUSED_SMPL_QUERY", "0") != "0"
    device_skip = os.environ.get("VT_DEVICE_SKIP", "1") != "0"

    def __init__(self, smpl_model, regressors, priors, decoders=None, part_labels=None, obj_verts=None, obj_faces=None, obj_points=None,
                 cam=ops.DEFAULT_CAM, device="cuda:0"):
        self.device = torch.device(device)
        dev = self.device
        self.smpl = ops.SmplhHandle(smpl_model, dev)
        self.b25 = ops.LandmarkHandle(regressors["body25"], dev)
        self.net = ops.SifNetHandle(decoders, cam, dev) if decoders is not None else None
        self.cam = np.ascontiguousarray(cam, np.float32)
        t = lambda a, dt=torch.float32: None if a is None else torch.as_tensor(np.ascontiguousarray(a), dtype=dt, device=dev)
        self.pri = {k: t(v) for k, v in priors.items()}
        self.labels = t(part_labels, torch.int32)
        self.vert_order = t(morton_order(np.asarray(smpl_model["v_template"])), torch.int32) if self.sort_query_points else None
        if obj_points is not None and self.sort_object_points:
            obj_points = np.asarray(obj_points, np.float32)[morton_order(obj_points)]
        self.obj_verts = t(obj_verts); self.obj_faces = t(obj_faces, torch.int32); self.obj_points = t(obj_points)
        self.smpl_faces = t(np.asarray(smpl_model["f"]).astype(np.int32), torch.int32) if "f" in smpl_model else None
        self.jw66 = t(JOINT_WEIGHTS_66)

    range_retries = 0
    fp32_fallbacks = 0
    _counter_lock = threading.Lock()
    host_wait_s = 0.0

    def _with_range_fallback(self, maps, params, run):
        if self.net is None or maps is None or maps.force_fp32 or self.net.precision == "fp32":
            return run()
        saved = [p.clone() for p in params]
        while True:
            try:
                return run()
            except FloatingPointError as e:
                import warnings
                for p, s0 in zip(params, saved):
                    p.copy_(s0)
                if maps.act_level + 1 < maps.ACT_LEVELS:
                    maps.set_act_level(maps.act_level + 1)
                    warnings.warn(f"{e}; repeating the fit at operand-range level {maps.act_level} of the split-f16 decoders", RuntimeWarning)
                    with self._counter_lock:
                        self.range_retries += 1
                    continue
                if maps.force_fp32:
                    raise
                warnings.warn(f"{e}; repeating the fit on the strict-fp32 decoder kernels (5x slower)", RuntimeWarning)
                maps.set_force_fp32(True)
                with self._counter_lock:
                    self.fp32_fallbacks += 1
                return run()

    def smpl_forward(self, pose, betas, trans, verts, jtr, vposed, ws):
        _chk(_lib().vt_smplh_forward(self.smpl.h, pose.data_ptr(), betas.data_ptr(), trans.data_ptr(), pose.shape[0], verts.data_ptr(),
                                     jtr.data_ptr(), vposed.data_ptr(), ws.data_ptr(), L.stream_ptr()))

    def smpl_backward(self, pose, betas, dverts, vposed, ws, scratch, dpose, dbetas, dtrans):
        _chk(_lib().vt_smplh_backward(self.smpl.h, pose.data_ptr(), betas.data_ptr(), pose.shape[0], dverts.data_ptr(), None, vposed.data_ptr(),
                                      ws.data_ptr(), scratch.data_ptr(), dpose.data_ptr(), dbetas.data_ptr(), dtrans.data_ptr(), L.stream_ptr()))

    def hand_prior_value(self, pose, terms, name, scratch_b):
        B = pose.shape[0]
        for off, m, p in ((66, "lhand_mean", "lhand_prec"), (111, "rhand_mean", "rhand_prec")):
            _chk(_lib().vt_mahalanobis(pose.data_ptr(), B, 156, off, 45, self.pri[m].data_ptr(), self.pri[p].data_ptr(), scratch_b.data_ptr(), None, 0.0, L.stream_ptr()))
            _chk(_lib().vt_sum_to_term(scratch_b.data_ptr(), B, 1.0 / 45.0, terms.ptr(name), L.stream_ptr()))

    def body_prior(self, pose, dpose, w, terms, name, scratch_b):
        B = pose.shape[0]
        _chk(_lib().vt_mahalanobis(pose.data_ptr(), B, 156, 3, 63, self.pri["body_mean"].data_ptr(), self.pri["body_prec"].data_ptr(),
                                   scratch_b.data_ptr(), dpose.data_ptr(), w / B, L.stream_ptr()))
        _chk(_lib().vt_sum_to_term(scratch_b.data_ptr(), B, 1.0 / B, terms.ptr(name), L.stream_ptr()))

    def _run_fit(self, f, start, end, check_every, outer, prof=None):
        res = FitResult()
        with self._skip_after_stop(f.stop) as skipping:
            watch = _StopWatch(self, f.stop, skipping)
            for it in range(start, end):
                step, phase, w, armed = outer(it)
                for i in range(10):
                    step(f, phase, (it - start) * 10 + i, w, armed)
                res.steps += 10
                res.outer_iters += 1
                if (it - start) % check_every == check_every - 1 and watch.check():
                    res.stopped_early = True
                    break
            res.stopped_early = res.stopped_early or watch.final()
        res.losses = f.hist.cpu().numpy()
        if res.stopped_early:
            res.steps = int(np.isfinite(res.losses).sum())
            res.outer_iters = -(-res.steps // 10)
        _flush_events(prof, f.lp, res.steps if (res.stopped_early and self.device_skip) else None)
        _check_finite(res, "fit")
        return res

    def fit_smplt(self, pose, betas, trans, kpts, max_iter=100, iter_for_global=8, temporal=True, pinit_w=900.0,
                  lr_global=0.01, lr_all=0.001, it_range=None, check_every=1, weights=None, early_stop=True):
        with torch.cuda.device(pose.device):
            return self._fit_smplt(pose, betas, trans, kpts, max_iter, iter_for_global, temporal, pinit_w, lr_global, lr_all, it_range, check_every, weights, early_stop)

    def _fit_smplt(self, pose, betas, trans, kpts, max_iter, iter_for_global, temporal, pinit_w, lr_global, lr_all, it_range, check_every, weights, early_stop=True):
        _require_params(pose, betas, trans)
        table = dict(SMPLT_WEIGHTS); table["pinit"] = pinit_w
        if weights is not None:
            table.update({k: float(v) for k, v in weights.items() if k in table})
        start, end = it_range if it_range is not None else (0, max_iter)
        f = _SmplFit(pose, betas, trans, ["kpts", "temp", "ptemp", "pose", "pinit", "hand"], (end - start) * 10, 0.0)
        f.kpts = _as_input(kpts, pose.device)
        f.temporal = temporal and f.B >= 3
        self.hand_prior_value(pose, f.terms, "hand", f.vb)

        def outer(it):
            if f.adam is None or it == iter_for_global:
                if it < iter_for_global:
                    f.adam = AdamState([(trans, 3, f.dtrans, lr_global), (pose, 3, f.dpose, lr_global), (betas, 2, f.dbetas, lr_global)], f.stop)
                else:
                    f.adam = AdamState([(trans, 3, f.dtrans, lr_all), (pose, 66, f.dpose, lr_all), (betas, 10, f.dbetas, lr_all)], f.stop)
            return self._smplt_step, None, f.terms.weights(table, it // 3), int(early_stop and it > 0.3 * max_iter)
        return self._run_fit(f, start, end, check_every, outer)

    def optimize_smpl(self, maps, pose, betas, trans, crop_center, body_center, body_kpts, max_iter=100, iter_for_betas=1,
                      iter_for_pose=1, iter_for_kpts=1, it_range=None, net_size=512.0, check_every=1, prof=None, early_stop=True):
        with torch.cuda.device(pose.device):
            return self._with_range_fallback(maps, (pose, betas, trans), lambda: self._optimize_smpl(
                maps, pose, betas, trans, crop_center, body_center, body_kpts, max_iter, iter_for_betas, iter_for_pose, iter_for_kpts, it_range, net_size,
                check_every, prof, early_stop))

    def _optimize_smpl(self, maps, pose, betas, trans, crop_center, body_center, body_kpts, max_iter, iter_for_betas, iter_for_pose, iter_for_kpts,
                       it_range, net_size, check_every, prof, early_stop=True):
        dev = pose.device
        _require_params(pose, betas, trans)
        split_route = self.net.precision != "fp32" and not maps.force_fp32
        if self.use_projection and split_route:
            maps.build_projection(self.net)
        total = iter_for_betas + iter_for_kpts + iter_for_pose + max_iter
        start, end = it_range if it_range is not None else (0, total)
        f = _SmplFit(pose, betas, trans, ["df_h", "part", "pose", "pinit", "j2d", "stemp", "hand"], (end - start) * 10, 300.0, prof)
        f.maps, f.net_size = maps, net_size
        f.crop_center, f.body_center, f.body_kpts = _as_input(crop_center, dev), _as_input(body_center, dev), _as_input(body_kpts, dev)
        f.vert_order = self.vert_order
        if self.sort_query_points:
            self.smpl_forward(pose, betas, trans, f.verts, f.jtr, f.vposed, f.ws)
            v0 = f.verts[f.B // 2]
            f.vert_order = morton_order_device(torch.stack([v0[:, 0] / v0[:, 2], v0[:, 1] / v0[:, 2]], 1))
        self.hand_prior_value(pose, f.terms, "hand", f.vb)
        if not self.fused_steps:
            step = self._smpl_step
        elif split_route and self.fused_smpl_query:
            step = self._smpl_step_fused_query
        else:
            step = self._smpl_step_fused
        arm_after = 0.25 * max_iter + iter_for_betas + iter_for_pose

        def outer(it):
            if it < iter_for_betas:
                phase = "global"
                if f.adam is None:
                    f.adam = AdamState([(betas, 2, f.dbetas, 0.02), (trans, 3, f.dtrans, 0.02)], f.stop)
            else:
                phase = "kpts" if it >= iter_for_betas + iter_for_pose else "smpl all pose"
                if f.adam is None or it == iter_for_betas:
                    f.adam = AdamState([(trans, 3, f.dtrans, 0.006), (pose, 66, f.dpose, 0.006), (betas, 10, f.dbetas, 0.006)], f.stop)
            return step, phase, f.terms.weights(FIT_WEIGHTS, 1 if phase != "kpts" else it / 3), int(early_stop and it > arm_after)
        return self._run_fit(f, start, end, check_every, outer, prof)

    def optimize_smpl_object(self, maps, smpl_verts, obj_R, obj_t, obj_s, crop_center, body_center, occ, sil=None, noise=None,
                             iter_for_obj=15, iter_for_sil=30, joint_iter=10, max_iter=100, it_range=None, seed=0, check_every=1, prof=None, early_stop=True):
        with torch.cuda.device(obj_R.device):
            return self._with_range_fallback(maps, (obj_R, obj_t), lambda: self._optimize_smpl_object(
                maps, smpl_verts, obj_R, obj_t, obj_s, crop_center, body_center, occ, sil, noise, iter_for_obj, iter_for_sil, joint_iter, max_iter, it_range,
                seed, check_every, prof, early_stop))

    def _optimize_smpl_object(self, maps, smpl_verts, obj_R, obj_t, obj_s, crop_center, body_center, occ, sil, noise, iter_for_obj, iter_for_sil,
                              joint_iter, max_iter, it_range, seed, check_every, prof, early_stop=True):
        dev = obj_R.device; B = obj_R.shape[0]
        _require_params(obj_R, obj_t)
        if self.use_projection and self.net.precision != "fp32" and not maps.force_fp32:
            maps.build_projection(self.net)
        total = joint_iter + iter_for_obj + max_iter + iter_for_sil
        start, end = it_range if it_range is not None else (0, total)
        f = _ObjectFit(self, obj_R, obj_t, sil, (end - start) * 10, prof)
        f.maps = maps
        f.smpl_verts, f.obj_s, f.crop_center, f.body_center, f.occ = (_as_input(x, dev) for x in (smpl_verts, obj_s, crop_center, body_center, occ))
        f.obj_s = f.obj_s.reshape(-1)
        if noise is not None:
            f.noise = _as_input(noise, dev)
        else:
            gen = torch.Generator(device=dev); gen.manual_seed(seed)
            f.noise = torch.rand((end - start) * 10, B, 3, 3, device=dev, generator=gen)
        ones = torch.ones_like(f.obj_s)
        _chk(_lib().vt_sqdiff_loss(f.obj_s.data_ptr(), 1, ones.data_ptr(), 1, B, 1, float(B), 0.0, f.terms.ptr("scale"), None, L.stream_ptr()))
        Rv, dMv = obj_R.view(B, 9), f.dM.view(B, 9)

        def outer(it):
            if it < iter_for_obj:
                phase = "object only"
                if f.adam is None:
                    f.adam = AdamState([(Rv, 9, dMv, 0.002), (obj_t, 3, f.dt, 0.006)], f.stop)
            elif it < iter_for_obj + iter_for_sil:
                phase = "sil"
                if sil is None:
                    raise L.VtError("phase 'sil' needs a SilSetup")
                if f.adam is None or it == iter_for_obj:
                    f.adam = AdamState([(Rv, 9, dMv, 0.006), (obj_t, 3, f.dt, 0.006)], f.stop)
                    f.trans_init = obj_t.clone()
            else:
                phase = "joint"
                if f.adam is None or it == iter_for_obj + iter_for_sil:
                    f.adam = AdamState([(obj_t, 3, f.dt, 0.002)], f.stop)
            decay = 1 if phase == "object only" else (it - iter_for_obj + 1 if phase == "sil" else (it - iter_for_obj + 1) / 3)
            tw = 10.0 if phase == "joint" else 1.0
            w = f.terms.weights(FIT_WEIGHTS, decay, {"otemp": tw, "ovtemp": tw})
            fused = self.fused_steps and not (phase == "joint" and self.collision_loss)
            return (self._object_step_fused if fused else self._object_step), phase, w, int(early_stop and phase == "joint" and it > 0.25 * max_iter)
        return self._run_fit(f, start, end, check_every, outer, prof)

    def _read_stop(self, stop):
        t0 = time.perf_counter()
        v = int(stop.item())
        with self._counter_lock:
            self.host_wait_s += time.perf_counter() - t0
        return v

    @contextlib.contextmanager
    def _skip_after_stop(self, stop):
        if not self.device_skip:
            yield False
            return
        sp = L.stream_ptr()
        rc = _lib().vt_stream_set_skip_flag(sp, stop.data_ptr())
        if rc == L.VT_ERR_BUSY:
            yield False
            return
        L.check(rc)
        try:
            yield True
        finally:
            _lib().vt_stream_set_skip_flag(sp, None)

    def _smplt_step(self, f, phase, k, w, armed):
        lib = _lib(); st = L.stream_ptr(); B = f.B; pose = f.pose
        f.terms.zero(0, 5)
        self.smpl_forward(pose, f.betas, f.trans, f.verts, f.jtr, f.vposed, f.ws)
        _chk(lib.vt_landmarks_forward(self.b25.h, f.verts.data_ptr(), B, f.J.data_ptr(), st))
        _chk(lib.vt_kpts_loss(f.J.data_ptr(), f.kpts.data_ptr(), None, B, 25, 0, self.cam.ctypes.data, 0.0, float(w[0]), f.terms.ptr("kpts"), f.dJ.data_ptr(), st))
        _chk(lib.vt_landmarks_backward(self.b25.h, f.dJ.data_ptr(), B, f.dverts.data_ptr(), 0, st))
        if f.temporal:
            _chk(lib.vt_accel_loss(f.verts.data_ptr(), B, 6890 * 3, None, float(w[1]), f.terms.ptr("temp"), f.dverts.data_ptr(), st))
        self.smpl_backward(pose, f.betas, f.dverts, f.vposed, f.ws, f.scratch, f.dpose, f.dbetas, f.dtrans)
        if f.temporal:
            _chk(lib.vt_accel_loss_strided(pose.data_ptr(), B, 66, 156, self.jw66.data_ptr(), float(w[2]), f.terms.ptr("ptemp"), f.dpose.data_ptr(), st))
        self.body_prior(pose, f.dpose, float(w[3]), f.terms, "pose", f.vb)
        _chk(lib.vt_sqdiff_loss(pose.data_ptr() + 12, 156, f.pose_init.data_ptr() + 12, 156, B, 63, float(B * 63), float(w[4]),
                                f.terms.ptr("pinit"), f.dpose.data_ptr() + 12, st))
        f.adam.step()
        _chk(lib.vt_loss_reduce_and_stop(f.terms.buf.data_ptr(), w.ctypes.data, len(f.terms.names), 1e-3, armed, f.loss_state.data_ptr(),
                                         f.stop.data_ptr(), f.hist.data_ptr(), k, st))

    def _human_query(self, f, k, w):
        ev = _ev_begin(f.lp)
        _chk(_lib().vt_query_human_loss(self.net.h, C.byref(f.maps.c), f.verts.data_ptr(), f.crop_center.data_ptr(), f.body_center.data_ptr(), f.B, 6890,
                                        self.labels.data_ptr(), f.vert_order_ptr, float(w[0]), float(w[1]), f.dverts.data_ptr(), f.terms.ptr("df_h"),
                                        L.stream_ptr()))
        _ev_end(f.lp, "human", ev, f.B, k)

    def _smpl_step(self, f, phase, k, w, armed):
        lib = _lib(); st = L.stream_ptr(); B = f.B; pose = f.pose
        f.terms.zero(0, 6)
        self.smpl_forward(pose, f.betas, f.trans, f.verts, f.jtr, f.vposed, f.ws)
        self._human_query(f, k, w)
        if phase == "kpts":
            _chk(lib.vt_landmarks_forward(self.b25.h, f.verts.data_ptr(), B, f.J.data_ptr(), st))
            _chk(lib.vt_kpts_loss(f.J.data_ptr(), f.body_kpts.data_ptr(), f.crop_center.data_ptr(), B, 25, 1, self.cam.ctypes.data, f.net_size,
                                  float(w[4]), f.terms.ptr("j2d"), f.dJ.data_ptr(), st))
            _chk(lib.vt_landmarks_backward(self.b25.h, f.dJ.data_ptr(), B, f.dverts.data_ptr(), 1, st))
        if B >= 4:
            _chk(lib.vt_accel_loss(f.verts.data_ptr(), B, 6890 * 3, None, float(w[5]), f.terms.ptr("stemp"), f.dverts.data_ptr(), st))
        self.smpl_backward(pose, f.betas, f.dverts, f.vposed, f.ws, f.scratch, f.dpose, f.dbetas, f.dtrans)
        self.body_prior(pose, f.dpose, float(w[2]), f.terms, "pose", f.vb)
        _chk(lib.vt_sqdiff_loss(pose.data_ptr() + 12, 156, f.pose_init.data_ptr() + 12, 156, B, 69, float(B), float(w[3]),
                                f.terms.ptr("pinit"), f.dpose.data_ptr() + 12, st))
        f.adam.step()
        _chk(lib.vt_loss_reduce_and_stop(f.terms.buf.data_ptr(), w.ctypes.data, len(f.terms.names), 1e-3, armed, f.loss_state.data_ptr(),
                                         f.stop.data_ptr(), f.hist.data_ptr(), k, st))

    def _smpl_step_fused(self, f, phase, k, w, armed):
        lib = _lib(); st = L.stream_ptr(); B = f.B
        self.smpl_forward(f.pose, f.betas, f.trans, f.verts, f.jtr, f.vposed, f.ws)
        self._human_query(f, k, w)
        if phase == "kpts":
            _chk(lib.vt_kpts_step(self.b25.h, f.verts.data_ptr(), f.body_kpts.data_ptr(), f.crop_center.data_ptr(), B, 1, self.cam.ctypes.data, f.net_size,
                                  float(w[4]), f.terms.ptr("j2d"), f.J.data_ptr(), f.dverts.data_ptr(), 1, st))
        if B >= 4:
            _chk(lib.vt_accel_loss(f.verts.data_ptr(), B, 6890 * 3, None, float(w[5]), f.terms.ptr("stemp"), f.dverts.data_ptr(), st))
        self.smpl_backward(f.pose, f.betas, f.dverts, f.vposed, f.ws, f.scratch, f.dpose, f.dbetas, f.dtrans)
        self._smpl_tail(f, k, w, armed)

    def _smpl_step_fused_query(self, f, phase, k, w, armed):
        lib = _lib(); st = L.stream_ptr(); B = f.B
        self.smpl_forward(f.pose, f.betas, f.trans, f.verts, f.jtr, f.vposed, f.ws)
        if phase == "kpts":
            _chk(lib.vt_kpts_step(self.b25.h, f.verts.data_ptr(), f.body_kpts.data_ptr(), f.crop_center.data_ptr(), B, 1, self.cam.ctypes.data, f.net_size,
                                  float(w[4]), f.terms.ptr("j2d"), f.J.data_ptr(), f.dverts.data_ptr(), 0, st))
        ev = _ev_begin(f.lp)
        _chk(lib.vt_query_human_step(self.net.h, C.byref(f.maps.c), f.verts.data_ptr(), f.crop_center.data_ptr(), f.body_center.data_ptr(), B, 6890,
                                     self.labels.data_ptr(), f.vert_order_ptr, float(w[0]), float(w[1]), int(phase == "kpts"), float(w[5]),
                                     f.terms.ptr("stemp") if B >= 4 else None, f.dverts.data_ptr(), f.terms.ptr("df_h"), st))
        _ev_end(f.lp, "human", ev, B, k)
        self.smpl_backward(f.pose, f.betas, f.dverts, f.vposed, f.ws, f.scratch, f.dpose, f.dbetas, f.dtrans)
        self._smpl_tail(f, k, w, armed)

    def _smpl_tail(self, f, k, w, armed):
        _chk(_lib().vt_smplstep_tail(f.pose.data_ptr(), f.pose_init.data_ptr(), f.dpose.data_ptr(), f.B, self.pri["body_mean"].data_ptr(),
                                     self.pri["body_prec"].data_ptr(), float(w[2]) / f.B, f.terms.ptr("pose"), float(w[3]), f.terms.ptr("pinit"),
                                     *f.adam.smpl_tail_groups, f.adam.tick(), 0.9, 0.999, 1e-8,
                                     f.terms.buf.data_ptr(), w.ctypes.data, len(f.terms.names), 1e-3, armed, f.loss_state.data_ptr(), f.stop.data_ptr(),
                                     f.hist.data_ptr(), k, f.ticket.data_ptr(), 6, L.stream_ptr()))

    def _object_query(self, f, k, w):
        ev = _ev_begin(f.lp)
        _chk(_lib().vt_query_object_loss(self.net.h, C.byref(f.maps.c), f.X.data_ptr(), f.crop_center.data_ptr(), f.body_center.data_ptr(), f.B, f.N,
                                         f.occ.data_ptr(), float(w[0]), f.dX.data_ptr(), f.terms.ptr("object"), L.stream_ptr()))
        _ev_end(f.lp, "object", ev, f.B, k)

    def _contacts(self, f, w):
        if f.contact is None:
            f.contact = self._contacts_once(f.maps, f.smpl_verts, f.X, f.crop_center, f.body_center)
        if f.contact["P"] > 0:
            self._contact_term(f.contact, f.X, f.dX, float(w[5]), f.terms)

    def _object_step(self, f, phase, k, w, armed):
        lib = _lib(); st = L.stream_ptr(); B, N, NV, nz = f.B, f.N, f.NV, f.noise[k]
        obj_R, obj_t, obj_s, X, dX, R, dR, dt = f.obj_R, f.obj_t, f.obj_s, f.X, f.dX, f.R, f.dR, f.dt
        nf = self.obj_faces.shape[0]
        f.terms.zero(0, 7)
        _chk(lib.vt_so3_project_forward(obj_R.data_ptr(), nz.data_ptr(), B, R.data_ptr(), st))
        _chk(lib.vt_rigid_forward(self.obj_points.data_ptr(), 1, R.data_ptr(), obj_t.data_ptr(), obj_s.data_ptr(), B, N, X.data_ptr(), st))
        if phase == "sil":
            _chk(lib.vt_fill(dX.data_ptr(), dX.numel(), 0.0, st))
        else:
            self._object_query(f, k, w)
        if B >= 4:
            _chk(lib.vt_accel_loss(X.data_ptr(), B, N * 3, None, float(w[1]), f.terms.ptr("otemp"), dX.data_ptr(), st))
            _chk(lib.vt_velocity_loss(X.data_ptr(), B, N * 3, float(w[2]), f.terms.ptr("ovtemp"), dX.data_ptr(), st))
        acc = 0
        if phase == "sil":
            sil = f.sil
            _chk(lib.vt_rigid_forward(self.obj_verts.data_ptr(), 1, R.data_ptr(), obj_t.data_ptr(), obj_s.data_ptr(), B, NV, f.Vt.data_ptr(), st))
            _chk(lib.vt_sil_forward(f.Vt.data_ptr(), B, NV, self.obj_faces.data_ptr(), nf, sil.K.data_ptr(), sil.size, f.img.data_ptr(), f.fidx.data_ptr(),
                                    f.sws.data_ptr(), st))
            _chk(lib.vt_sil_mask_loss(f.img.data_ptr(), sil.keep.data_ptr(), sil.ref.data_ptr(), f.occ.data_ptr(), B, sil.size, float(w[3]),
                                      f.terms.ptr("mask"), f.per.data_ptr(), f.dimg.data_ptr(), st))
            _chk(lib.vt_sil_backward(f.Vt.data_ptr(), B, NV, self.obj_faces.data_ptr(), nf, sil.K.data_ptr(), sil.size, f.fidx.data_ptr(), f.dimg.data_ptr(),
                                     1e-4, f.sws.data_ptr(), f.dVt.data_ptr(), st))
            _chk(lib.vt_rigid_backward(self.obj_verts.data_ptr(), 1, obj_s.data_ptr(), B, NV, f.dVt.data_ptr(), dR.data_ptr(), dt.data_ptr(), 0, st))
            _chk(lib.vt_sqdiff_loss(obj_t.data_ptr(), 3, f.trans_init.data_ptr(), 3, B, 3, float(B * 3), float(w[4]), f.terms.ptr("trans"), dt.data_ptr(), st))
            acc = 1
        if phase == "joint":
            self._contacts(f, w)
        _chk(lib.vt_rigid_backward(self.obj_points.data_ptr(), 1, obj_s.data_ptr(), B, N, dX.data_ptr(), dR.data_ptr(), dt.data_ptr(), acc, st))
        if phase == "joint" and self.collision_loss:
            if f.cws is None:
                f.Vc = torch.empty(B, NV, 3, device=X.device)
                f.cws = torch.empty((lib.vt_collision_workspace_bytes(B, self.smpl_faces.shape[0]) + 7) // 8, dtype=torch.int64, device=X.device)
            _chk(lib.vt_rigid_forward(self.obj_verts.data_ptr(), 1, R.data_ptr(), obj_t.data_ptr(), obj_s.data_ptr(), B, NV, f.Vc.data_ptr(), st))
            _chk(lib.vt_collision_loss(f.smpl_verts.data_ptr(), f.smpl_verts.shape[1], self.smpl_faces.data_ptr(), self.smpl_faces.shape[0], f.Vc.data_ptr(), NV,
                                       self.obj_faces.data_ptr(), nf, B, 0.5, 8, float(w[6]), f.terms.ptr("collide"), dt.data_ptr(), None, f.cws.data_ptr(), st))
        _chk(lib.vt_so3_project_backward(obj_R.data_ptr(), nz.data_ptr(), B, dR.data_ptr(), f.dM.data_ptr(), st))
        f.adam.step()
        _chk(lib.vt_loss_reduce_and_stop(f.terms.buf.data_ptr(), w.ctypes.data, len(f.terms.names), 1e-4, armed, f.loss_state.data_ptr(), f.stop.data_ptr(),
                                         f.hist.data_ptr(), k, st))

    def _object_step_fused(self, f, phase, k, w, armed):
        lib = _lib(); st = L.stream_ptr(); B, N, NV, nz = f.B, f.N, f.NV, f.noise[k]
        is_sil = phase == "sil"
        X, dX = f.X.data_ptr(), f.dX.data_ptr()
        obj_verts, Vt, dVt = (self.obj_verts.data_ptr(), f.Vt.data_ptr(), f.dVt.data_ptr()) if is_sil else (None, None, None)
        _chk(lib.vt_objstep_head(f.obj_R.data_ptr(), nz.data_ptr(), f.obj_t.data_ptr(), f.obj_s.data_ptr(), B, self.obj_points.data_ptr(), N, X,
                                 obj_verts, NV, Vt, f.R.data_ptr(), f.terms.buf.data_ptr(), 7, f.svd_ws.data_ptr(), st))
        if not is_sil:
            self._object_query(f, k, w)
        tail_temporal = B >= 4 and phase != "joint"
        if B >= 4 and phase == "joint":
            _chk(lib.vt_temporal_loss2(X, B, N * 3, float(w[1]), f.terms.ptr("otemp"), float(w[2]), f.terms.ptr("ovtemp"), dX, 0, st))
        elif is_sil and B < 4:
            _chk(lib.vt_fill(dX, f.dX.numel(), 0.0, st))
        if is_sil:
            sil = f.sil
            _chk(lib.vt_sil_step(Vt, B, NV, self.obj_faces.data_ptr(), self.obj_faces.shape[0], sil.K.data_ptr(), sil.size, sil.keep.data_ptr(),
                                 sil.ref.data_ptr(), f.occ.data_ptr(), float(w[3]), 1e-4, f.terms.ptr("mask"), f.fidx.data_ptr(), f.dimg.data_ptr(),
                                 f.sws.data_ptr(), dVt, st))
        if phase == "joint":
            self._contacts(f, w)
        tail, pre = lib.vt_objstep_tail, ()
        if tail_temporal:
            tail, pre = lib.vt_objstep_tail_temporal, (X, float(w[1]), f.terms.ptr("otemp"), float(w[2]), f.terms.ptr("ovtemp"), int(is_sil))
        _chk(tail(*pre, obj_verts, NV, dVt, self.obj_points.data_ptr(), N, dX, f.obj_s.data_ptr(), B, f.obj_R.data_ptr(), nz.data_ptr(), f.obj_t.data_ptr(),
                  f.trans_init.data_ptr() if is_sil else None, float(w[4]), f.terms.ptr("trans"), f.dR.data_ptr(), f.dt.data_ptr(), f.dM.data_ptr(),
                  *f.adam.object_tail_groups, f.adam.tick(), 0.9, 0.999, 1e-8, f.terms.buf.data_ptr(), w.ctypes.data, len(f.terms.names), 1e-4, armed,
                  f.loss_state.data_ptr(), f.stop.data_ptr(), f.hist.data_ptr(), k, f.ticket.data_ptr(), 0, f.svd_ws.data_ptr(), st))

    def _contact_term(self, contact, X, dX, w, terms):
        _chk(_lib().vt_chamfer_ragged_idx(contact["x"].data_ptr(), contact["offx"].data_ptr(), contact["x"].shape[0], X.data_ptr(), contact["idx_o32"].data_ptr(),
                                          contact["offy"].data_ptr(), contact["idx_o32"].shape[0], contact["P"], w, terms.ptr("contact"), dX.data_ptr(),
                                          contact["ws"].data_ptr(), int(not contact["planned"]), L.stream_ptr()))
        contact["planned"] = True

    def _contacts_once(self, maps, smpl_verts, X, crop_center, body_center, thres=0.08):
        B, N = X.shape[:2]; V = smpl_verts.shape[1]; dev = X.device
        df_o, _, parts_o, _, _ = ops.sifnet_query(self.net, maps, X, crop_center, body_center, head_mask=0b00101)
        df_h, _, _, _, _ = ops.sifnet_query(self.net, maps, smpl_verts, crop_center, body_center, head_mask=0b00001)
        mask_o = df_o[:, 0] < thres
        mask_h = df_h[:, 1] < thres
        lab_o = parts_o.argmax(1)
        lab_h = self.labels.long().unsqueeze(0).expand(B, V)
        oh = torch.zeros(B, 14, device=dev, dtype=torch.long); oo = torch.zeros_like(oh)
        oh.scatter_add_(1, lab_h, mask_h.long()); oo.scatter_add_(1, lab_o, mask_o.long())
        pair = (oh > 0) & (oo > 0)
        P = int(pair.sum().item())
        if P == 0:
            return {"P": 0}
        sel_h = mask_h & pair.gather(1, lab_h); sel_o = mask_o & pair.gather(1, lab_o)
        bh, vh = sel_h.nonzero(as_tuple=True); bo, no = sel_o.nonzero(as_tuple=True)
        cnt_h = (oh * pair).reshape(-1); cnt_o = (oo * pair).reshape(-1)
        keep = pair.reshape(-1)
        ch, co = cnt_h[keep], cnt_o[keep]
        perm = torch.argsort(ch * co, descending=True, stable=True)
        rank_of_key = torch.zeros(B * 14, dtype=torch.long, device=dev)
        rank_of_key[keep.nonzero(as_tuple=True)[0][perm]] = torch.arange(P, device=dev)
        kh = rank_of_key[bh * 14 + lab_h[bh, vh]]; ko = rank_of_key[bo * 14 + lab_o[bo, no]]
        oh_s = torch.sort(kh, stable=True); oo_s = torch.sort(ko, stable=True)
        idx_h = (bh * V + vh)[oh_s.indices]; idx_o = (bo * N + no)[oo_s.indices]
        offx = torch.zeros(P + 1, dtype=torch.int32, device=dev); offy = torch.zeros(P + 1, dtype=torch.int32, device=dev)
        offx[1:] = torch.cumsum(ch[perm], 0).int(); offy[1:] = torch.cumsum(co[perm], 0).int()
        x = smpl_verts.reshape(-1, 3).index_select(0, idx_h).contiguous()
        ws = torch.empty(int(_lib().vt_chamfer_ws_bytes(x.shape[0], idx_o.shape[0], P)), dtype=torch.uint8, device=dev)
        return {"P": P, "x": x, "offx": offx, "offy": offy, "idx_o": idx_o, "idx_o32": idx_o.int().contiguous(), "ws": ws, "planned": False}


class SilSetup:

    def __init__(self, K, keep, ref, size=256):
        self.K, self.keep, self.ref, self.size = K.contiguous(), keep.contiguous(), ref.contiguous(), size
```

Measured before the change: 152.8.

## Precompute frozen hand-joint pose blend contribution once per fit and skip it per step

Only the first 22 body joints are optimized (Adam updates 66 pose columns), so the rotation and pose-blend GEMM contribution of the frozen hand joints is constant within a fit. A new fix-tail pass computes those rotations and the partial vertex offsets once per fit. The per-step forward then loads the precomputed offsets and runs the MFMA loop only over the free-joint and beta K-slices. The backward skips blend tiles, part reductions and rodrigues backward for the frozen joints. This cuts the large pose-blend GEMM work per iteration, at the cost of extra workspace, template variants and an assumption that hand poses stay fixed during the fit.

```diff
diff --git a/include/vistracker.h b/include/vistracker.h
--- a/include/vistracker.h
+++ b/include/vistracker.h
@@ -35,6 +35,14 @@
 int vt_smplh_backward(const vt_smplh *h, const float *pose, const float *betas, int B, const float *dverts,
                       const float *djtr, const float *v_posed, const float *ws, float *scratch,
                       float *dpose, float *dbetas, float *dtrans, void *stream);
+
+long vt_smplh_fix_floats(int B);
+int vt_smplh_fix_tail(const vt_smplh *h, const float *pose, int B, int n_free_joints, float *fix, void *stream);
+int vt_smplh_forward_fixed(const vt_smplh *h, const float *pose, const float *betas, const float *trans, int B, int n_free_joints,
+                           const float *fix, int fix_B, float *verts, float *jtr, float *v_posed, float *ws, void *stream);
+int vt_smplh_backward_fixed(const vt_smplh *h, const float *pose, const float *betas, int B, int n_free_joints, const float *dverts,
+                            const float *djtr, const float *v_posed, const float *ws, float *scratch,
+                            float *dpose, float *dbetas, float *dtrans, void *stream);
 
 int vt_rodrigues_forward(const float *aa, int n, float *R, void *stream);
 int vt_rodrigues_backward(const float *aa, int n, const float *dR, float *daa, void *stream);
diff --git a/vistracker_amd/_lib.py b/vistracker_amd/_lib.py
--- a/vistracker_amd/_lib.py
+++ b/vistracker_amd/_lib.py
@@ -28,6 +28,10 @@
     "vt_smplh_bwd_scratch_floats": (cl, [ci]),
     "vt_smplh_forward": (ci, [vp, fp, fp, fp, ci, fp, fp, fp, fp, vp]),
     "vt_smplh_backward": (ci, [vp, fp, fp, ci, fp, fp, fp, fp, fp, fp, fp, fp, vp]),
+    "vt_smplh_fix_floats": (cl, [ci]),
+    "vt_smplh_fix_tail": (ci, [vp, fp, ci, ci, fp, vp]),
+    "vt_smplh_forward_fixed": (ci, [vp, fp, fp, fp, ci, ci, fp, ci, fp, fp, fp, fp, vp]),
+    "vt_smplh_backward_fixed": (ci, [vp, fp, fp, ci, ci, fp, fp, fp, fp, fp, fp, fp, fp, vp]),
     "vt_rodrigues_forward": (ci, [fp, ci, fp, vp]),
     "vt_rodrigues_backward": (ci, [fp, ci, fp, fp, vp]),
     "vt_landmarks_create": (ci, [C.POINTER(vp), vp, vp, vp, ci, ci, vp]),
diff --git a/vistracker_amd/csrc/smplh.hip b/vistracker_amd/csrc/smplh.hip
--- a/vistracker_amd/csrc/smplh.hip
+++ b/vistracker_amd/csrc/smplh.hip
@@ -98,7 +98,8 @@
 __global__ __launch_bounds__(64) void smplh_pose_kernel(const float *__restrict__ pose, const float *__restrict__ betas,
                                                         const float *__restrict__ trans, const float *__restrict__ J_t,
                                                         const float *__restrict__ J_s, SmplParents par,
-                                                        float *__restrict__ ws, float *__restrict__ jtr, const int *skip)
+                                                        float *__restrict__ ws, float *__restrict__ jtr, const int *skip,
+                                                        const float *__restrict__ fixR, int n_free)
 {
     VT_SKIP_RETURN(skip);
     __shared__ float sR[J_ * 9], sJ[J_ * 3], sG[J_ * 12];
@@ -106,7 +107,11 @@
     float *w = ws + (size_t)b * WS_FRAME;
     if (j < J_) {
         float t[3] = {pose[(b * J_ + j) * 3], pose[(b * J_ + j) * 3 + 1], pose[(b * J_ + j) * 3 + 2]}, R[9];
-        rodrigues_fwd(t, R, nullptr);
+        if (fixR != nullptr && j >= n_free) {
+#pragma unroll
+            for (int e = 0; e < 9; e++) R[e] = fixR[((size_t)b * J_ + j) * 9 + e];
+        } else
+            rodrigues_fwd(t, R, nullptr);
 #pragma unroll
         for (int e = 0; e < 9; e++) { sR[j * 9 + e] = R[e]; w[WS_R + j * 9 + e] = R[e]; }
 #pragma unroll
@@ -164,10 +169,13 @@
 #define AXS 516
 #define SAS 628
 #define FWD_R0 (FWD_FB * AXS > 8 * SAS ? FWD_FB * AXS : 8 * SAS)
+struct FwdTail { const float *Hin; float *Hout; const float *rot; int rot_stride, kf, nlo, shi, send; };
+template <int MODE>
 __global__ __launch_bounds__(256) void smplh_verts_kernel(const float *__restrict__ Q_kcv, const float *__restrict__ W_jv,
                                                           const float *__restrict__ betas, const float *__restrict__ trans,
                                                           const float *__restrict__ ws, int B,
-                                                          float *__restrict__ verts, float *__restrict__ v_posed, const float *__restrict__ W_sp, int nnz, const int *skip)
+                                                          float *__restrict__ verts, float *__restrict__ v_posed, const float *__restrict__ W_sp, int nnz, const int *skip,
+                                                          FwdTail ft)
 {
     VT_SKIP_RETURN(skip);
     extern __shared__ __attribute__((aligned(16))) float lds[];
@@ -182,6 +190,14 @@
         const int e9 = k % 9;
         const float sub = (k < NP_ && (e9 == 0 || e9 == 4 || e9 == 8)) ? 1.f : 0.f;
         float val[FWD_FB];
+        if (MODE == 2) {
+            const bool keep = k >= ft.kf && k < NP_;
+#pragma unroll
+            for (int f = 0; f < FWD_FB; f++) val[f] = keep ? ft.rot[(size_t)min(b0 + f, B - 1) * ft.rot_stride + 9 + k] - sub : 0.f;
+#pragma unroll
+            for (int f = 0; f < FWD_FB; f++) sAx[f * AXS + k] = val[f];
+            continue;
+        }
 #pragma unroll
         for (int f = 0; f < FWD_FB; f++) {
             const int b = min(b0 + f, B - 1);
@@ -189,17 +205,19 @@
             else if (k < NP_ + NB_) val[f] = betas[b * NB_ + (k - NP_)];
             else val[f] = (k == NP_ + NB_) ? 1.f : 0.f;
         }
-#pragma unroll
-        for (int f = 0; f < FWD_FB; f++) sAx[f * AXS + k] = val[f] - sub;
-    }
-    if (nnz > 0) {
+        const bool keep = MODE == 0 || k < ft.kf || k >= NP_;
+#pragma unroll
+        for (int f = 0; f < FWD_FB; f++) sAx[f * AXS + k] = keep ? val[f] - sub : 0.f;
+    }
+    if (MODE == 2) {
+    } else if (nnz > 0) {
         for (int i = tid; i < nnz * 64; i += 256) {
             sW[i] = W_sp[(size_t)(i >> 6) * VP_ + blockIdx.x * 64 + (i & 63)];
             sW[SP_K * 64 + i] = W_sp[(size_t)(SP_K + (i >> 6)) * VP_ + blockIdx.x * 64 + (i & 63)];
         }
     } else
         for (int i = tid; i < J_ * 64; i += 256) sW[i] = W_jv[(i >> 6) * VP_ + blockIdx.x * 64 + (i & 63)];
-    if (tid < FWD_FB * 3) { const int f = tid / 3, b = min(b0 + f, B - 1); sTr[tid] = trans[b * 3 + tid % 3]; }
+    if (MODE != 2 && tid < FWD_FB * 3) { const int f = tid / 3, b = min(b0 + f, B - 1); sTr[tid] = trans[b * 3 + tid % 3]; }
     __syncthreads();
 
     f32x4 acc[3];
@@ -213,19 +231,59 @@
         _Pragma("unroll") for (int e = 0; e < 2; e++)                                            \
             _Pragma("unroll") for (int c = 0; c < 3; c++) bq[slot_][e][c] = qk[(size_t)(e * 3 + c) * VP_]; \
     }
-#pragma unroll
-    for (int s = 0; s < FWD_PF; s++) FWD_LOADQ(s, s)
-#pragma unroll
-    for (int s = 0; s < NS; s++) {
-        const float2 av = *reinterpret_cast<const float2 *>(sAx + j * AXS + 8 * s + 2 * q);
-#pragma unroll
-        for (int c = 0; c < 3; c++) acc[c] = MFMA16(av.x, bq[s % FWD_PF][0][c], acc[c]);
-#pragma unroll
-        for (int c = 0; c < 3; c++) acc[c] = MFMA16(av.y, bq[s % FWD_PF][1][c], acc[c]);
-        if (s + FWD_PF < NS) FWD_LOADQ(s % FWD_PF, s + FWD_PF)
-        __builtin_amdgcn_sched_barrier(0);
+    if (MODE == 0) {
+#pragma unroll
+        for (int s = 0; s < FWD_PF; s++) FWD_LOADQ(s, s)
+#pragma unroll
+        for (int s = 0; s < NS; s++) {
+            const float2 av = *reinterpret_cast<const float2 *>(sAx + j * AXS + 8 * s + 2 * q);
+#pragma unroll
+            for (int c = 0; c < 3; c++) acc[c] = MFMA16(av.x, bq[s % FWD_PF][0][c], acc[c]);
+#pragma unroll
+            for (int c = 0; c < 3; c++) acc[c] = MFMA16(av.y, bq[s % FWD_PF][1][c], acc[c]);
+            if (s + FWD_PF < NS) FWD_LOADQ(s % FWD_PF, s + FWD_PF)
+            __builtin_amdgcn_sched_barrier(0);
+        }
+    } else {
+        const int nlo = ft.nlo, shi = ft.shi, n = nlo + ft.send - shi;
+#pragma unroll
+        for (int u = 0; u < FWD_PF; u++)
+            if (u < n) { const int s = u < nlo ? u : shi + u - nlo; FWD_LOADQ(u, s) }
+        if (MODE == 1) {
+#pragma unroll
+            for (int r = 0; r < 4; r++)
+#pragma unroll
+                for (int c = 0; c < 3; c++) acc[c][r] = v < V_ ? ft.Hin[((size_t)min(b0 + 4 * q + r, B - 1) * V_ + v) * 3 + c] : 0.f;
+        }
+#pragma unroll 1
+        for (int i0 = 0; i0 < n; i0 += FWD_PF) {
+#pragma unroll
+            for (int u = 0; u < FWD_PF; u++) {
+                const int i = i0 + u;
+                if (i < n) {
+                    const int s = i < nlo ? i : shi + i - nlo;
+                    const float2 av = *reinterpret_cast<const float2 *>(sAx + j * AXS + 8 * s + 2 * q);
+#pragma unroll
+                    for (int c = 0; c < 3; c++) acc[c] = MFMA16(av.x, bq[u][0][c], acc[c]);
+#pragma unroll
+                    for (int c = 0; c < 3; c++) acc[c] = MFMA16(av.y, bq[u][1][c], acc[c]);
+                    if (i + FWD_PF < n) { const int i2 = i + FWD_PF, s2 = i2 < nlo ? i2 : shi + i2 - nlo; FWD_LOADQ(u, s2) }
+                }
+                __builtin_amdgcn_sched_barrier(0);
+            }
+        }
     }
 #undef FWD_LOADQ
+    if (MODE == 2) {
+#pragma unroll
+        for (int r = 0; r < 4; r++) {
+            const int b = b0 + 4 * q + r;
+            if (b < B && v < V_)
+#pragma unroll
+                for (int c = 0; c < 3; c++) ft.Hout[((size_t)b * V_ + v) * 3 + c] = acc[c][r];
+        }
+        return;
+    }
     __syncthreads();
 #pragma unroll
     for (int r = 0; r < 4; r++)
@@ -372,13 +430,17 @@
 #define BL_NW 1
 #endif
 #define BL_AS 132
+#define BL_T_BETAS (NP_ / 16)
 __global__ __launch_bounds__(256) void smplh_bwd_blend_kernel(const float *__restrict__ Q_p, const float *__restrict__ dvp_g, int B,
-                                                              float *__restrict__ part3, const int *skip)
+                                                              float *__restrict__ part3, const int *skip, int nlo_t, int ntiles)
 {
     VT_SKIP_RETURN(skip);
     __shared__ __attribute__((aligned(16))) float sA[BL_M * BL_AS];
     const int tid = threadIdx.x, wave = tid >> 6, lane = tid & 63, q = lane >> 4, j = lane & 15;
-    const int ks = blockIdx.x, m0 = blockIdx.z * BL_M, nt0 = blockIdx.y * (4 * BL_NW) + wave * BL_NW;
+    const int ks = blockIdx.x, m0 = blockIdx.z * BL_M, lt0 = blockIdx.y * (4 * BL_NW) + wave * BL_NW;
+    int nt[BL_NW];
+#pragma unroll
+    for (int n = 0; n < BL_NW; n++) { const int lt = min(lt0 + n, ntiles - 1); nt[n] = lt < nlo_t ? lt : BL_T_BETAS + lt - nlo_t; }
     f32x4 acc[6][BL_NW];
 #pragma unroll
     for (int mt = 0; mt < 6; mt++)
@@ -395,13 +457,14 @@
             *reinterpret_cast<float4 *>(sA + row * BL_AS + c4 * 4) = v;
         }
         __syncthreads();
+        if (lt0 >= ntiles) continue;
 #pragma unroll
         for (int g = 0; g < 8; g++) {
             const size_t kg = (size_t)ks * KG_SLAB + c * 8 + g;
             float bq[BL_NW][4];
 #pragma unroll
             for (int n = 0; n < BL_NW; n++) {
-                const float4 fq = Q4[(kg * (NQ_ / 16) + min(nt0 + n, NQ_ / 16 - 1)) * 64 + lane];
+                const float4 fq = Q4[(kg * (NQ_ / 16) + nt[n]) * 64 + lane];
                 bq[n][0] = fq.x; bq[n][1] = fq.y; bq[n][2] = fq.z; bq[n][3] = fq.w;
             }
 #pragma unroll
@@ -424,7 +487,7 @@
                 float *dst = part3 + ((size_t)ks * B + b) * NQ_;
 #pragma unroll
                 for (int n = 0; n < BL_NW; n++)
-                    if (nt0 + n < NQ_ / 16) dst[(nt0 + n) * 16 + j] = acc[mt][n][r];
+                    if (lt0 + n < ntiles) dst[nt[n] * 16 + j] = acc[mt][n][r];
             }
         }
     }
@@ -434,7 +497,7 @@
                                                               SmplParents par, const float *__restrict__ ws,
                                                               const float *__restrict__ part, const float *__restrict__ part3,
                                                               const float *__restrict__ djtr, int B, float *__restrict__ dpose, float *__restrict__ dbetas,
-                                                              float *__restrict__ dtrans, const int *skip)
+                                                              float *__restrict__ dtrans, const int *skip, int n_free)
 {
     VT_SKIP_RETURN(skip);
     __shared__ float red[PT_N], red3[NQ_];
@@ -453,8 +516,10 @@
     }
     for (int i = tid; i < NQ_; i += 256) {
         float s = 0.f;
+        if (i < 9 * (n_free - 1) || (i >= NP_ && i < NP_ + NB_)) {
 #pragma unroll 9
-        for (int t = 0; t < NKS_; t++) s += part3[((size_t)t * B + b) * NQ_ + i];
+            for (int t = 0; t < NKS_; t++) s += part3[((size_t)t * B + b) * NQ_ + i];
+        }
         red3[i] = s;
     }
     __syncthreads();
@@ -505,10 +570,10 @@
     __syncthreads();
     if (tid < J_) {
         const int j = tid;
-        float g[9], t[3] = {pose[(b * J_ + j) * 3], pose[(b * J_ + j) * 3 + 1], pose[(b * J_ + j) * 3 + 2]}, d[3];
+        float g[9], t[3] = {pose[(b * J_ + j) * 3], pose[(b * J_ + j) * 3 + 1], pose[(b * J_ + j) * 3 + 2]}, d[3] = {0.f, 0.f, 0.f};
 #pragma unroll
         for (int e = 0; e < 9; e++) g[e] = sdR[9 * j + e] + (j >= 1 ? red3[(j - 1) * 9 + e] : 0.f);
-        rodrigues_bwd(t, g, d);
+        if (j < n_free) rodrigues_bwd(t, g, d);
         dpose[(b * J_ + j) * 3] = d[0]; dpose[(b * J_ + j) * 3 + 1] = d[1]; dpose[(b * J_ + j) * 3 + 2] = d[2];
     } else if (tid >= 64 && tid < 64 + NB_) {
         const int l = tid - 64;
@@ -609,38 +674,111 @@
 
 #define BWD_FB 6
 
+__global__ void smplh_fix_rot_kernel(const float *__restrict__ pose, int n, int n_free, float *__restrict__ R)
+{
+    const int i = blockIdx.x * blockDim.x + threadIdx.x;
+    if (i >= n) return;
+    float t[3] = {pose[3 * i], pose[3 * i + 1], pose[3 * i + 2]}, r[9] = {0.f, 0.f, 0.f, 0.f, 0.f, 0.f, 0.f, 0.f, 0.f};
+    if (i % J_ >= n_free) rodrigues_fwd(t, r, nullptr);
+#pragma unroll
+    for (int e = 0; e < 9; e++) R[9 * i + e] = r[e];
+}
+
+#define FIX_H_FLOATS(B_) ((size_t)(B_) * V_ * 3)
+extern "C" long vt_smplh_fix_floats(int B) { return (long)(FIX_H_FLOATS(B) + (size_t)B * J_ * 9); }
+
+static int smplh_forward_launch(const vt_smplh *h, const float *pose, const float *betas, const float *trans, int B, int n_free, const float *fix,
+                                float *verts, float *jtr, float *v_posed, float *ws, hipStream_t st)
+{
+    const int *skip = vt_skip_flag_of(st);
+    const float *fixR = fix ? fix + FIX_H_FLOATS(B) : nullptr;
+    hipLaunchKernelGGL(smplh_pose_kernel, dim3(B), dim3(64), 0, st, pose, betas, trans, h->J_t, h->J_s, h->par, ws, jtr, skip, fixR, n_free);
+    VT_LAUNCH_CHECK();
+    const size_t lds_f = sizeof(float) * (FWD_R0 + FWD_FB * 64 * 3 + (h->nnz > 0 ? 2 * SP_K * 64 : J_ * 64) + FWD_FB * 3);
+    const size_t lds_max = sizeof(float) * (FWD_R0 + FWD_FB * 64 * 3 + J_ * 64 + FWD_FB * 3);
+    const dim3 grid(VP_ / 64, (B + FWD_FB - 1) / FWD_FB);
+    if (fix) {
+        const int kf = 9 * (n_free - 1), s_betas = NP_ / 8;
+        const FwdTail ft = {fix, nullptr, nullptr, 0, kf, std::min((kf + 7) / 8, s_betas), s_betas, KQ_ / 8};
+        VT_LDS_LIMIT(smplh_verts_kernel<1>, lds_max);
+        hipLaunchKernelGGL(smplh_verts_kernel<1>, grid, dim3(256), lds_f, st, h->Q_kcv, h->W_jv, betas, trans, ws, B, verts, v_posed, h->W_sp, h->nnz, skip, ft);
+    } else {
+        const FwdTail ft = {nullptr, nullptr, nullptr, 0, NP_, 0, 0, 0};
+        VT_LDS_LIMIT(smplh_verts_kernel<0>, lds_max);
+        hipLaunchKernelGGL(smplh_verts_kernel<0>, grid, dim3(256), lds_f, st, h->Q_kcv, h->W_jv, betas, trans, ws, B, verts, v_posed, h->W_sp, h->nnz, skip, ft);
+    }
+    VT_LAUNCH_CHECK();
+    return VT_OK;
+}
+
 extern "C" int vt_smplh_forward(const vt_smplh *h, const float *pose, const float *betas, const float *trans, int B,
                                 float *verts, float *jtr, float *v_posed, float *ws, void *stream)
 {
     VT_REQUIRE(h && pose && betas && trans && verts && v_posed && ws && B > 0, "vt_smplh_forward: null argument or B <= 0");
-    hipStream_t st = vt_stream(stream); const int *skip = vt_skip_flag_of(st);
-    hipLaunchKernelGGL(smplh_pose_kernel, dim3(B), dim3(64), 0, st, pose, betas, trans, h->J_t, h->J_s, h->par, ws, jtr, skip);
-    VT_LAUNCH_CHECK();
-    const size_t lds_f = sizeof(float) * (FWD_R0 + FWD_FB * 64 * 3 + (h->nnz > 0 ? 2 * SP_K * 64 : J_ * 64) + FWD_FB * 3);
-    VT_LDS_LIMIT(smplh_verts_kernel, sizeof(float) * (FWD_R0 + FWD_FB * 64 * 3 + J_ * 64 + FWD_FB * 3));
-    hipLaunchKernelGGL(smplh_verts_kernel, dim3(VP_ / 64, (B + FWD_FB - 1) / FWD_FB), dim3(256), lds_f, st, h->Q_kcv, h->W_jv, betas, trans, ws, B,
-                       verts, v_posed, h->W_sp, h->nnz, skip);
-    VT_LAUNCH_CHECK();
-    return VT_OK;
-}
-
-extern "C" int vt_smplh_backward(const vt_smplh *h, const float *pose, const float *betas, int B, const float *dverts,
-                                 const float *djtr, const float *v_posed, const float *ws, float *scratch,
-                                 float *dpose, float *dbetas, float *dtrans, void *stream)
-{
-    (void)betas;
-    VT_REQUIRE(h && pose && dverts && v_posed && ws && scratch && dpose && dbetas && dtrans && B > 0, "vt_smplh_backward: null argument or B <= 0");
-    hipStream_t st = vt_stream(stream); const int *skip = vt_skip_flag_of(st);
+    return smplh_forward_launch(h, pose, betas, trans, B, J_, nullptr, verts, jtr, v_posed, ws, vt_stream(stream));
+}
+
+static int smplh_backward_launch(const vt_smplh *h, const float *pose, int B, int n_free, const float *dverts, const float *djtr, const float *v_posed,
+                                 const float *ws, float *scratch, float *dpose, float *dbetas, float *dtrans, hipStream_t st)
+{
+    const int *skip = vt_skip_flag_of(st);
     const size_t lds = sizeof(float) * (256 * 13 + BWD_FB * 624);
     float *dvp_g = scratch + (size_t)NVT_ * B * PT_N, *part3 = dvp_g + (size_t)B * KTOT_;
     VT_LDS_LIMIT(smplh_bwd_tile_kernel<BWD_FB>, lds);
     hipLaunchKernelGGL(smplh_bwd_tile_kernel<BWD_FB>, dim3(NVT_, (B + BWD_FB - 1) / BWD_FB), dim3(256), lds, st, h->W_v64, ws, v_posed, dverts, B, scratch, dvp_g, skip);
     VT_LAUNCH_CHECK();
-    hipLaunchKernelGGL(smplh_bwd_blend_kernel, dim3(NKS_, (NQ_ / 16 + 4 * BL_NW - 1) / (4 * BL_NW), (B + BL_M - 1) / BL_M), dim3(256), 0, st, h->Q_t, dvp_g, B, part3, skip);
-    VT_LAUNCH_CHECK();
-    hipLaunchKernelGGL(smplh_bwd_frame_kernel, dim3(B), dim3(256), 0, st, pose, h->J_s, h->par, ws, scratch, part3, djtr, B, dpose, dbetas, dtrans, skip);
+    const int nlo_t = std::min((9 * (n_free - 1) + 15) / 16, BL_T_BETAS), ntiles = nlo_t + NQ_ / 16 - BL_T_BETAS;
+    hipLaunchKernelGGL(smplh_bwd_blend_kernel, dim3(NKS_, (ntiles + 4 * BL_NW - 1) / (4 * BL_NW), (B + BL_M - 1) / BL_M), dim3(256), 0, st, h->Q_t, dvp_g, B, part3, skip,
+                       nlo_t, ntiles);
+    VT_LAUNCH_CHECK();
+    hipLaunchKernelGGL(smplh_bwd_frame_kernel, dim3(B), dim3(256), 0, st, pose, h->J_s, h->par, ws, scratch, part3, djtr, B, dpose, dbetas, dtrans, skip, n_free);
     VT_LAUNCH_CHECK();
     return VT_OK;
+}
+
+extern "C" int vt_smplh_backward(const vt_smplh *h, const float *pose, const float *betas, int B, const float *dverts,
+                                 const float *djtr, const float *v_posed, const float *ws, float *scratch,
+                                 float *dpose, float *dbetas, float *dtrans, void *stream)
+{
+    (void)betas;
+    VT_REQUIRE(h && pose && dverts && v_posed && ws && scratch && dpose && dbetas && dtrans && B > 0, "vt_smplh_backward: null argument or B <= 0");
+    return smplh_backward_launch(h, pose, B, J_, dverts, djtr, v_posed, ws, scratch, dpose, dbetas, dtrans, vt_stream(stream));
+}
+
+extern "C" int vt_smplh_fix_tail(const vt_smplh *h, const float *pose, int B, int n_free_joints, float *fix, void *stream)
+{
+    VT_REQUIRE(h && pose && fix && B > 0, "vt_smplh_fix_tail: null argument or B <= 0");
+    VT_REQUIRE(n_free_joints >= 1 && n_free_joints <= J_, "vt_smplh_fix_tail: n_free_joints = %d outside 1..%d", n_free_joints, J_);
+    hipStream_t st = vt_stream(stream);
+    float *fixR = fix + FIX_H_FLOATS(B);
+    hipLaunchKernelGGL(smplh_fix_rot_kernel, dim3((B * J_ + 255) / 256), dim3(256), 0, st, pose, B * J_, n_free_joints, fixR);
+    VT_LAUNCH_CHECK();
+    const int kf = 9 * (n_free_joints - 1);
+    const FwdTail ft = {nullptr, fix, fixR, J_ * 9, kf, 0, kf / 8, (NP_ + 7) / 8};
+    VT_LDS_LIMIT(smplh_verts_kernel<2>, sizeof(float) * FWD_R0);
+    hipLaunchKernelGGL(smplh_verts_kernel<2>, dim3(VP_ / 64, (B + FWD_FB - 1) / FWD_FB), dim3(256), sizeof(float) * FWD_R0, st, h->Q_kcv, nullptr, nullptr, nullptr,
+                       nullptr, B, nullptr, nullptr, nullptr, 0, nullptr, ft);
+    VT_LAUNCH_CHECK();
+    return VT_OK;
+}
+
+extern "C" int vt_smplh_forward_fixed(const vt_smplh *h, const float *pose, const float *betas, const float *trans, int B, int n_free_joints,
+                                      const float *fix, int fix_B, float *verts, float *jtr, float *v_posed, float *ws, void *stream)
+{
+    VT_REQUIRE(h && pose && betas && trans && fix && verts && v_posed && ws && B > 0, "vt_smplh_forward_fixed: null argument or B <= 0");
+    VT_REQUIRE(n_free_joints >= 1 && n_free_joints <= J_, "vt_smplh_forward_fixed: n_free_joints = %d outside 1..%d", n_free_joints, J_);
+    VT_REQUIRE(fix_B == B, "vt_smplh_forward_fixed: the fixed-tail buffer was built for B = %d, not %d", fix_B, B);
+    return smplh_forward_launch(h, pose, betas, trans, B, n_free_joints, n_free_joints < J_ ? fix : nullptr, verts, jtr, v_posed, ws, vt_stream(stream));
+}
+
+extern "C" int vt_smplh_backward_fixed(const vt_smplh *h, const float *pose, const float *betas, int B, int n_free_joints, const float *dverts,
+                                       const float *djtr, const float *v_posed, const float *ws, float *scratch,
+                                       float *dpose, float *dbetas, float *dtrans, void *stream)
+{
+    (void)betas;
+    VT_REQUIRE(h && pose && dverts && v_posed && ws && scratch && dpose && dbetas && dtrans && B > 0, "vt_smplh_backward_fixed: null argument or B <= 0");
+    VT_REQUIRE(n_free_joints >= 1 && n_free_joints <= J_, "vt_smplh_backward_fixed: n_free_joints = %d outside 1..%d", n_free_joints, J_);
+    return smplh_backward_launch(h, pose, B, n_free_joints, dverts, djtr, v_posed, ws, scratch, dpose, dbetas, dtrans, vt_stream(stream));
 }
 
 extern "C" int vt_rodrigues_forward(const float *aa, int n, float *R, void *stream)
diff --git a/vistracker_amd/fitting.py b/vistracker_amd/fitting.py
--- a/vistracker_amd/fitting.py
+++ b/vistracker_amd/fitting.py
@@ -20,6 +20,7 @@
 SMPLT_WEIGHTS = {"pose": 1e-5, "hand": 1e-5, "kpts": 0.09, "temp": 900.0, "ptemp": 25.0, "pinit": 900.0}
 JOINT_WEIGHTS_66 = np.repeat(np.array([1, 10, 10, 10, 5, 5, 10, 1, 1, 10, 1, 1, 5, 5, 5, 5, 5, 5, 1, 1, 1, 1], np.float32), 3)
 JOINT_WEIGHTS_66[37:39] = 10.0
+FREE_POSE_COLS = 66
 
 
 def _lib():
@@ -222,6 +223,7 @@
         self.dpose = torch.empty(B, 156, device=dev); self.dbetas = torch.empty(B, 10, device=dev); self.dtrans = torch.empty(B, 3, device=dev)
         self.vb = torch.empty(B, device=dev)
         self.pose_init = pose.clone()
+        self.fix = None
 
     @property
     def vert_order_ptr(self):
@@ -256,6 +258,7 @@
     fused_steps = os.environ.get("VT_FUSED_STEPS", "1") != "0"
     fused_smpl_query = os.environ.get("VT_FUSED_SMPL_QUERY", "0") != "0"
     device_skip = os.environ.get("VT_DEVICE_SKIP", "1") != "0"
+    fixed_hands = os.environ.get("VT_SMPLH_FIXED_HANDS", "0") != "0"
 
     def __init__(self, smpl_model, regressors, priors, decoders=None, part_labels=None, obj_verts=None, obj_faces=None, obj_points=None,
                  cam=ops.DEFAULT_CAM, device="cuda:0"):
@@ -305,11 +308,30 @@
                     self.fp32_fallbacks += 1
                 return run()
 
-    def smpl_forward(self, pose, betas, trans, verts, jtr, vposed, ws):
-        _chk(_lib().vt_smplh_forward(self.smpl.h, pose.data_ptr(), betas.data_ptr(), trans.data_ptr(), pose.shape[0], verts.data_ptr(),
+    def smpl_fix_tail(self, pose):
+        if not self.fixed_hands:
+            return None
+        B = pose.shape[0]
+        fix = torch.empty(B, _lib().vt_smplh_fix_floats(B) // B, device=pose.device)
+        _chk(_lib().vt_smplh_fix_tail(self.smpl.h, pose.data_ptr(), B, FREE_POSE_COLS // 3, fix.data_ptr(), L.stream_ptr()))
+        return fix
+
+    def smpl_forward(self, pose, betas, trans, verts, jtr, vposed, ws, fix=None):
+        B = pose.shape[0]
+        if fix is not None:
+            _chk(_lib().vt_smplh_forward_fixed(self.smpl.h, pose.data_ptr(), betas.data_ptr(), trans.data_ptr(), B, FREE_POSE_COLS // 3, fix.data_ptr(),
+                                               fix.shape[0], verts.data_ptr(), jtr.data_ptr(), vposed.data_ptr(), ws.data_ptr(),
+                                               L.stream_ptr()))
+            return
+        _chk(_lib().vt_smplh_forward(self.smpl.h, pose.data_ptr(), betas.data_ptr(), trans.data_ptr(), B, verts.data_ptr(),
                                      jtr.data_ptr(), vposed.data_ptr(), ws.data_ptr(), L.stream_ptr()))
 
-    def smpl_backward(self, pose, betas, dverts, vposed, ws, scratch, dpose, dbetas, dtrans):
+    def smpl_backward(self, pose, betas, dverts, vposed, ws, scratch, dpose, dbetas, dtrans, fix=None):
+        if fix is not None:
+            _chk(_lib().vt_smplh_backward_fixed(self.smpl.h, pose.data_ptr(), betas.data_ptr(), pose.shape[0], FREE_POSE_COLS // 3, dverts.data_ptr(), None,
+                                                vposed.data_ptr(), ws.data_ptr(), scratch.data_ptr(), dpose.data_ptr(), dbetas.data_ptr(), dtrans.data_ptr(),
+                                                L.stream_ptr()))
+            return
         _chk(_lib().vt_smplh_backward(self.smpl.h, pose.data_ptr(), betas.data_ptr(), pose.shape[0], dverts.data_ptr(), None, vposed.data_ptr(),
                                       ws.data_ptr(), scratch.data_ptr(), dpose.data_ptr(), dbetas.data_ptr(), dtrans.data_ptr(), L.stream_ptr()))
 
@@ -361,6 +383,7 @@
         f = _SmplFit(pose, betas, trans, ["kpts", "temp", "ptemp", "pose", "pinit", "hand"], (end - start) * 10, 0.0)
         f.kpts = _as_input(kpts, pose.device)
         f.temporal = temporal and f.B >= 3
+        f.fix = self.smpl_fix_tail(pose)
         self.hand_prior_value(pose, f.terms, "hand", f.vb)
 
         def outer(it):
@@ -368,7 +391,7 @@
                 if it < iter_for_global:
                     f.adam = AdamState([(trans, 3, f.dtrans, lr_global), (pose, 3, f.dpose, lr_global), (betas, 2, f.dbetas, lr_global)], f.stop)
                 else:
-                    f.adam = AdamState([(trans, 3, f.dtrans, lr_all), (pose, 66, f.dpose, lr_all), (betas, 10, f.dbetas, lr_all)], f.stop)
+                    f.adam = AdamState([(trans, 3, f.dtrans, lr_all), (pose, FREE_POSE_COLS, f.dpose, lr_all), (betas, 10, f.dbetas, lr_all)], f.stop)
             return self._smplt_step, None, f.terms.weights(table, it // 3), int(early_stop and it > 0.3 * max_iter)
         return self._run_fit(f, start, end, check_every, outer)
 
@@ -396,6 +419,7 @@
             self.smpl_forward(pose, betas, trans, f.verts, f.jtr, f.vposed, f.ws)
             v0 = f.verts[f.B // 2]
             f.vert_order = morton_order_device(torch.stack([v0[:, 0] / v0[:, 2], v0[:, 1] / v0[:, 2]], 1))
+        f.fix = self.smpl_fix_tail(pose)
         self.hand_prior_value(pose, f.terms, "hand", f.vb)
         if not self.fused_steps:
             step = self._smpl_step
@@ -413,7 +437,7 @@
             else:
                 phase = "kpts" if it >= iter_for_betas + iter_for_pose else "smpl all pose"
                 if f.adam is None or it == iter_for_betas:
-                    f.adam = AdamState([(trans, 3, f.dtrans, 0.006), (pose, 66, f.dpose, 0.006), (betas, 10, f.dbetas, 0.006)], f.stop)
+                    f.adam = AdamState([(trans, 3, f.dtrans, 0.006), (pose, FREE_POSE_COLS, f.dpose, 0.006), (betas, 10, f.dbetas, 0.006)], f.stop)
             return step, phase, f.terms.weights(FIT_WEIGHTS, 1 if phase != "kpts" else it / 3), int(early_stop and it > arm_after)
         return self._run_fit(f, start, end, check_every, outer, prof)
 
@@ -494,13 +518,13 @@
     def _smplt_step(self, f, phase, k, w, armed):
         lib = _lib(); st = L.stream_ptr(); B = f.B; pose = f.pose
         f.terms.zero(0, 5)
-        self.smpl_forward(pose, f.betas, f.trans, f.verts, f.jtr, f.vposed, f.ws)
+        self.smpl_forward(pose, f.betas, f.trans, f.verts, f.jtr, f.vposed, f.ws, f.fix)
         _chk(lib.vt_landmarks_forward(self.b25.h, f.verts.data_ptr(), B, f.J.data_ptr(), st))
         _chk(lib.vt_kpts_loss(f.J.data_ptr(), f.kpts.data_ptr(), None, B, 25, 0, self.cam.ctypes.data, 0.0, float(w[0]), f.terms.ptr("kpts"), f.dJ.data_ptr(), st))
         _chk(lib.vt_landmarks_backward(self.b25.h, f.dJ.data_ptr(), B, f.dverts.data_ptr(), 0, st))
         if f.temporal:
             _chk(lib.vt_accel_loss(f.verts.data_ptr(), B, 6890 * 3, None, float(w[1]), f.terms.ptr("temp"), f.dverts.data_ptr(), st))
-        self.smpl_backward(pose, f.betas, f.dverts, f.vposed, f.ws, f.scratch, f.dpose, f.dbetas, f.dtrans)
+        self.smpl_backward(pose, f.betas, f.dverts, f.vposed, f.ws, f.scratch, f.dpose, f.dbetas, f.dtrans, f.fix)
         if f.temporal:
             _chk(lib.vt_accel_loss_strided(pose.data_ptr(), B, 66, 156, self.jw66.data_ptr(), float(w[2]), f.terms.ptr("ptemp"), f.dpose.data_ptr(), st))
         self.body_prior(pose, f.dpose, float(w[3]), f.terms, "pose", f.vb)
@@ -520,7 +544,7 @@
     def _smpl_step(self, f, phase, k, w, armed):
         lib = _lib(); st = L.stream_ptr(); B = f.B; pose = f.pose
         f.terms.zero(0, 6)
-        self.smpl_forward(pose, f.betas, f.trans, f.verts, f.jtr, f.vposed, f.ws)
+        self.smpl_forward(pose, f.betas, f.trans, f.verts, f.jtr, f.vposed, f.ws, f.fix)
         self._human_query(f, k, w)
         if phase == "kpts":
             _chk(lib.vt_landmarks_forward(self.b25.h, f.verts.data_ptr(), B, f.J.data_ptr(), st))
@@ -529,7 +553,7 @@
             _chk(lib.vt_landmarks_backward(self.b25.h, f.dJ.data_ptr(), B, f.dverts.data_ptr(), 1, st))
         if B >= 4:
             _chk(lib.vt_accel_loss(f.verts.data_ptr(), B, 6890 * 3, None, float(w[5]), f.terms.ptr("stemp"), f.dverts.data_ptr(), st))
-        self.smpl_backward(pose, f.betas, f.dverts, f.vposed, f.ws, f.scratch, f.dpose, f.dbetas, f.dtrans)
+        self.smpl_backward(pose, f.betas, f.dverts, f.vposed, f.ws, f.scratch, f.dpose, f.dbetas, f.dtrans, f.fix)
         self.body_prior(pose, f.dpose, float(w[2]), f.terms, "pose", f.vb)
         _chk(lib.vt_sqdiff_loss(pose.data_ptr() + 12, 156, f.pose_init.data_ptr() + 12, 156, B, 69, float(B), float(w[3]),
                                 f.terms.ptr("pinit"), f.dpose.data_ptr() + 12, st))
@@ -539,19 +563,19 @@
 
     def _smpl_step_fused(self, f, phase, k, w, armed):
         lib = _lib(); st = L.stream_ptr(); B = f.B
-        self.smpl_forward(f.pose, f.betas, f.trans, f.verts, f.jtr, f.vposed, f.ws)
+        self.smpl_forward(f.pose, f.betas, f.trans, f.verts, f.jtr, f.vposed, f.ws, f.fix)
         self._human_query(f, k, w)
         if phase == "kpts":
             _chk(lib.vt_kpts_step(self.b25.h, f.verts.data_ptr(), f.body_kpts.data_ptr(), f.crop_center.data_ptr(), B, 1, self.cam.ctypes.data, f.net_size,
                                   float(w[4]), f.terms.ptr("j2d"), f.J.data_ptr(), f.dverts.data_ptr(), 1, st))
         if B >= 4:
             _chk(lib.vt_accel_loss(f.verts.data_ptr(), B, 6890 * 3, None, float(w[5]), f.terms.ptr("stemp"), f.dverts.data_ptr(), st))
-        self.smpl_backward(f.pose, f.betas, f.dverts, f.vposed, f.ws, f.scratch, f.dpose, f.dbetas, f.dtrans)
+        self.smpl_backward(f.pose, f.betas, f.dverts, f.vposed, f.ws, f.scratch, f.dpose, f.dbetas, f.dtrans, f.fix)
         self._smpl_tail(f, k, w, armed)
 
     def _smpl_step_fused_query(self, f, phase, k, w, armed):
         lib = _lib(); st = L.stream_ptr(); B = f.B
-        self.smpl_forward(f.pose, f.betas, f.trans, f.verts, f.jtr, f.vposed, f.ws)
+        self.smpl_forward(f.pose, f.betas, f.trans, f.verts, f.jtr, f.vposed, f.ws, f.fix)
         if phase == "kpts":
             _chk(lib.vt_kpts_step(self.b25.h, f.verts.data_ptr(), f.body_kpts.data_ptr(), f.crop_center.data_ptr(), B, 1, self.cam.ctypes.data, f.net_size,
                                   float(w[4]), f.terms.ptr("j2d"), f.J.data_ptr(), f.dverts.data_ptr(), 0, st))
@@ -560,7 +584,7 @@
                                      self.labels.data_ptr(), f.vert_order_ptr, float(w[0]), float(w[1]), int(phase == "kpts"), float(w[5]),
                                      f.terms.ptr("stemp") if B >= 4 else None, f.dverts.data_ptr(), f.terms.ptr("df_h"), st))
         _ev_end(f.lp, "human", ev, B, k)
-        self.smpl_backward(f.pose, f.betas, f.dverts, f.vposed, f.ws, f.scratch, f.dpose, f.dbetas, f.dtrans)
+        self.smpl_backward(f.pose, f.betas, f.dverts, f.vposed, f.ws, f.scratch, f.dpose, f.dbetas, f.dtrans, f.fix)
         self._smpl_tail(f, k, w, armed)
 
     def _smpl_tail(self, f, k, w, armed):
```

New measurement: 152.4 (median of 2 runs). Within noise of the previous version (-0.3%).
